# JADGardner/neusky

Hardware: AMD Instinct MI355X
Metric: train rays/sec on NeRF-OSR lk2 @1024 rays x 96 samples (higher is better)
Workload: dtype f32 in memory; forward products: fp16 hi + residual split, 3 x v_mfma_f32_32x32x16_f16 per product on power-of-two pre-scaled operands, one fp32 accumulator (~2^-22): FiLM-SIREN chains and the SDF / albedo field alike; backward products: the same fp16 split on per-row / per-matrix pre-scaled gradien; 1 GPU; full NeuSky train step (BASELINE configs[2]): 1024 rays/GPU x 96 samples, proposal 256+96, 512 illumination directions (256 upper-hemisphere DDF queries/ray), illumination decoder = this project's FiLM-SIREN H = 128 (RENI-shaped: latent 100x3; the reference's configured Attention decoder is absent from its tree), hash L16 F2 T2^19 x2, 256-wide MLPs; fwd + losses + bwd + all-reduce + 5 Adam groups; rays_per_gpu=1024, samples_per_ray=96, illumination_directions=512, parallelism=ray-sharded dp1, launcher=self-spawned, launch=HIP graph replay (1 graph/step + all-reduce + 5 Adam launches)

## Files before the change

### include/neusky_hip.h

```cpp
#ifndef NEUSKY_HIP_H
#define NEUSKY_HIP_H

#include <stdint.h>

#ifdef __cplusplus
extern "C" {
#endif

typedef void* nsky_stream_t;

const char* nsky_last_error(void);
int nsky_abi_version(void);

enum {
  NSKY_EPI_NONE = 0,
  NSKY_EPI_RELU = 1,
  NSKY_EPI_LEAKY = 2,
  NSKY_EPI_SIGMOID = 3,
  NSKY_EPI_SOFTPLUS = 4,
  NSKY_EPI_FILM = 5,
  NSKY_EPI_MUL_AUX = 6,
  NSKY_EPI_BWD_RELU = 7,
  NSKY_EPI_BWD_LEAKY = 8,
  NSKY_EPI_BWD_FILM = 9,
  NSKY_EPI_EXP = 10
};

enum { NSKY_PREC_F32 = 0, NSKY_PREC_BF16X2 = 2, NSKY_PREC_BF16X3 = 3, NSKY_PREC_F16X2 = 4 };

typedef struct nsky_gemm_desc {
  const float* A; const float* B; float* C;
  int32_t M, N, K;
  int32_t lda, ldb, ldc;
  int32_t a_kcontig, b_kcontig;
  const float* bias;
  int32_t epi;
  float p0, p1;
  const float* aux0; int32_t ldaux0;
  const float* aux1; int32_t ldaux1;
  const float* aux2; int32_t ldaux2;
  float* out1; int32_t ldout1;
  float* out2; int32_t ldout2;
  int32_t row_mod;
  int32_t k_splits;
  float beta;
  float* a_rowsum;
  int32_t precision;
  int32_t rowsum_k_limit;
  int32_t a_native_nt, b_native_nt;
  const float* a_scale_max;
} nsky_gemm_desc;

int nsky_gemm_f32(const nsky_gemm_desc* d, nsky_stream_t stream);

int nsky_split_planes(const float* W, int32_t n_rows, int32_t n_k, int32_t ldw, int32_t transpose, int32_t precision,
                      uint16_t* hi, uint16_t* lo, int32_t rows_pad, int32_t ldp, nsky_stream_t stream);
int nsky_gemm_f32_planes(const nsky_gemm_desc* d, const uint16_t* B_hi, const uint16_t* B_lo, int32_t ldp, nsky_stream_t stream);

int nsky_colsum_f32(const float* X, int32_t M, int32_t N, int32_t ldx, float* out, nsky_stream_t stream);
int nsky_weighted_colsum_f32(const float* X, int32_t M, int32_t N, int32_t ldx, const float* w, int32_t w_stride, float* out,
                             nsky_stream_t stream);

#define NSKY_FILM_MAX_LAYERS 12
#define NSKY_FILM_TABLE_FLOATS 6656
typedef struct nsky_film_net {
  int32_t hidden, n_map, n_film;
  int32_t cond_dim, x_dim, out_dim;
  const float* map_w[NSKY_FILM_MAX_LAYERS]; const float* map_b[NSKY_FILM_MAX_LAYERS]; int32_t map_ld[NSKY_FILM_MAX_LAYERS];
  const float* mo_w; const float* mo_b; int32_t mo_ld;
  const float* film_w[NSKY_FILM_MAX_LAYERS]; const float* film_b[NSKY_FILM_MAX_LAYERS]; int32_t film_ld[NSKY_FILM_MAX_LAYERS];
  const float* out_w; const float* out_b; int32_t out_ld;
} nsky_film_net;
int nsky_film_stream_layout(const nsky_film_net* net, int32_t direction, int64_t* stream_bytes, int32_t* n_tiles);
int nsky_film_pack(const nsky_film_net* net, int32_t direction, void* stream_buf, float* table, nsky_stream_t stream);
int nsky_film_chain_fwd(const nsky_film_net* net, const void* stream_buf, const float* table, const float* cond,
                        int32_t ldcond, const float* x, int32_t ldx, int32_t M, float* const* h_save, float* const* z_save,
                        float* const* y_save, float* res, int32_t ldres, nsky_stream_t stream);
int nsky_film_chain_bwd_film(const nsky_film_net* net, const void* stream_buf, const float* table, int32_t M, const float* d_res,
                             int32_t ldres, const float* h_last, const float* const* z_save, float* const* dz_save, float* dfp,
                             float* dfp_rowmax, float* gmax, float* d_x, int32_t ldx, nsky_stream_t stream);
int nsky_film_chain_bwd_map(const nsky_film_net* net, const void* stream_buf, const float* table, int32_t M, const float* dfp,
                            const float* dfp_rowmax, const float* const* h_save, float* const* dpre_save, float* d_cond,
                            int32_t ldcond, float* gmax, nsky_stream_t stream);
typedef struct {
  int32_t in_dim, hidden;
  const float* w0; int32_t ld0; const float* b0;
  const float* w1; int32_t ld1; const float* b1;
  const float* w2; const float* b2;
  float beta;
} nsky_sdf_net;
int nsky_sdf_stream_layout(const nsky_sdf_net* net, int32_t direction, int64_t* stream_bytes, int32_t* n_tiles);
int nsky_sdf_pack(const nsky_sdf_net* net, int32_t direction, void* stream_buf, float* table, nsky_stream_t stream);
int nsky_sdf_chain_fwd(const nsky_sdf_net* net, const void* stream_buf, const float* table, const float* E, int32_t ldE, int32_t M,
                       float* a0_save, float* a1_save, float* sdf, nsky_stream_t stream);
int nsky_sdf_chain_bwd(const nsky_sdf_net* net, const void* stream_buf, const float* table, int32_t M, const float* g_sdf,
                       const float* a0_save, const float* a1_save, float* dz1, float* dz0, float* dE, int32_t ldE, float* dw2,
                       float* db2, float* gmax, nsky_stream_t stream);

int nsky_wgrad_native(const float* dZ, int32_t nnt_a, const float* X, int32_t nnt_b, int32_t rows, float* dW, int32_t ldw,
                      float* db, const float* a_scale_max, float b_scale, nsky_stream_t stream);
#define NSKY_WGRAD_MAX_PROBLEMS 16
typedef struct {
  const float* dZ; int32_t nnt_a;
  const float* X;  int32_t nnt_b;
  float* dW;       int32_t ldw;
  float* db;
  const float* a_scale_max;
  float b_scale;
  int32_t lda, ldb, width_a, width_b, bias_rows;
  int32_t bias_row_mod;
  const float* b_scale_max;
} nsky_wgrad_problem;
int nsky_wgrad_native_batch(const nsky_wgrad_problem* problems, int32_t n_problems, int32_t rows, nsky_stream_t stream);

#define NSKY_CHAIN_MAX_LAYERS 8
typedef struct { const float* W; int32_t ld, rows, K, transposed; } nsky_chain_layer;
int nsky_chain_stream_layout(const nsky_chain_layer* layers, int32_t n_layers, int64_t* stream_bytes, int32_t* n_tiles, int32_t* n_groups);
int nsky_chain_pack(const nsky_chain_layer* layers, int32_t n_layers, void* stream_buf, float* scales, nsky_stream_t stream);
typedef struct nsky_field_net {
  int32_t in_dim;
  int32_t npe;
  float beta;
  const float* b0; const float* b1;
  const float* w_sdf; const float* b_sdf;
  const float* b2f;
  const float* bc0; const float* bc1;
  const float* wc2; int32_t ldc2; const float* bc2;
} nsky_field_net;
int nsky_field_geo_fwd(const nsky_field_net* net, const void* stream_buf, const float* scales, int32_t total_groups, const float* ET,
                       int32_t ldE, int32_t N, float* a0q, float* a1q, float* Eq, float* a1max, float* sdf, float* grad, float* qmax,
                       nsky_stream_t stream);
int nsky_field_colour_fwd(const nsky_field_net* net, const void* stream_buf, const float* scales, int32_t total_groups, const float* ET,
                          int32_t ldE, int32_t N, const float* a1q, const float* a1max, float* a1v, float* feat, float* xpe, float* c0, float* c1,
                          float* alb, nsky_stream_t stream);
int nsky_field_colour_bwd(const nsky_field_net* net, const void* stream_buf, const float* scales, int32_t total_groups, int32_t N,
                          const float* g_alb, const float* alb, const float* c0, const float* c1, float* dpc2, float* dpc1, float* dpc0,
                          float* dfeat, float* dxpe, float* da1v, float* gmax, nsky_stream_t stream);
int nsky_field_geo_bwd(const nsky_field_net* net, const void* stream_buf, const float* scales, int32_t total_groups, int32_t N,
                       const float* g_sdf, const float* g_grad, const float* da1v, const float* dxpe, const float* a0q, const float* a1q,
                       float* d1q, float* d0q, float* dET, int32_t ldE, float* gmax, nsky_stream_t stream);
int nsky_native_weighted_colsum(const float* X, int32_t nt, int32_t rows, const float* w4, int32_t n_out, const float* g_sdf,
                                const float* g_grad, float* out, int32_t ldo, float* bias, nsky_stream_t stream);
int nsky_field_geo_fwd_dir(const nsky_field_net* net, const void* stream_buf, const float* scales, int32_t total_groups, const float* ET,
                           int32_t ldE, int32_t N, float* a0q, float* a1q, float* Eq, float* sdf, float* cosv, float* qmax,
                           nsky_stream_t stream);
int nsky_field_geo_bwd_dir(const nsky_field_net* net, const void* stream_buf, const float* scales, int32_t total_groups, int32_t N,
                           const float* g_sdf, const float* g_cos, const float* a0q, const float* a1q, float* d1q, float* d0q, float* dET,
                           int32_t ldE, float* gmax, nsky_stream_t stream);
int nsky_native_weighted_colsum_pair(const float* X, int32_t nt, int32_t rows, const float* g_sdf, const float* g_cos, float* out,
                                     int32_t ldo, float* bias, nsky_stream_t stream);

int nsky_ray_reduce_fwd(const float* weights, const float* starts, const float* ends, const float* normals, const float* albedo,
                        int32_t R, int32_t S, float max_clamp, float* sums, float* bounds, float* p2p, float* accumulation,
                        float* normal, float* albedo_acc, nsky_stream_t stream);
int nsky_ray_reduce_bwd(const float* weights, const float* starts, const float* ends, const float* normals, const float* albedo,
                        const float* sums, const float* bounds, int32_t R, int32_t S, float max_clamp, const float* d_p2p,
                        const float* d_accumulation, const float* d_normal, const float* d_albedo_acc, float* d_weights,
                        float* d_normals, float* d_albedo, nsky_stream_t stream);


int nsky_point_alphas_fwd(const float* sdf, const float* grad, const float* dirs, const float* gap3_host, const float* variance, float anneal,
                          int32_t P, float* alphas, nsky_stream_t stream);
int nsky_point_alphas_bwd(const float* sdf, const float* grad, const float* dirs, const float* gap3_host, const float* variance, float anneal,
                          int32_t P, const float* d_alphas, float* d_sdf, float* d_grad, float* d_variance, nsky_stream_t stream);

int nsky_sigmoid_column_fwd(const float* raw, int32_t ld, int64_t n, float scale, float* t, nsky_stream_t stream);
int nsky_sigmoid_column_bwd(const float* raw, int32_t ld, int64_t n, float scale, const float* d_t, float* d_raw, nsky_stream_t stream);

int nsky_proposal_mlp_fwd(const float* feat, int32_t ldf, int64_t P, int32_t in_dim, int32_t hidden, const float* w0, int32_t ldw0,
                          const float* b0, const float* w1, const float* b1, float* raw, nsky_stream_t stream);
int nsky_proposal_mlp_bwd(const float* feat, int32_t ldf, int64_t P, int32_t in_dim, int32_t hidden, const float* w0, int32_t ldw0,
                          const float* b0, const float* w1, const float* b1, const float* d_raw, float* d_feat, float* dw0, float* db0,
                          float* dw1, float* db1, nsky_stream_t stream);
int nsky_ray_points_fwd(const float* origins, const float* dirs, int32_t n_dirs, float sign, const float* t, int64_t n, float* out,
                        nsky_stream_t stream);
int nsky_ray_points_bwd(const float* dirs, int32_t n_dirs, float sign, const float* d_out, int64_t n, float* d_t, nsky_stream_t stream);
int nsky_normalize3_fwd(const float* g, int64_t P, float* n, nsky_stream_t stream);
int nsky_normalize3_bwd(const float* g, const float* d_n, int64_t P, float* d_g, nsky_stream_t stream);

int nsky_ddf_vmf_samples(int32_t n_positions, int32_t n_directions, float kappa, float radius, int32_t upper_hemisphere,
                         uint64_t seed, uint64_t* counter, float* origins, float* directions, nsky_stream_t stream);

int nsky_ddf_fit_rows_fwd(const float* positions, const float* directions, const float* term_dist, int32_t N,
                          const float* mv_points_in, uint64_t seed, uint64_t* counter, const float* sky_o, const float* sky_d,
                          int32_t Ns, float radius, int32_t want_mv, float weight_exp, int32_t weight_include_z, float* q_pos,
                          float* xrow, int32_t ldx, float* mv_points_out, float* sky_gt, float* distance_weight, nsky_stream_t stream);
int nsky_ddf_fit_rows_bwd(const float* positions, const float* directions, const float* term_dist, const float* mv_points,
                          int32_t N, const float* d_xrow_mv, int32_t ldx, float* d_term_dist, nsky_stream_t stream);


int nsky_grid_probe_points(const float* lattice, const float* gap3_host, int32_t P, uint64_t seed, uint64_t* counter, float* positions,
                           float* directions, nsky_stream_t stream);

int nsky_reni_output_fwd(const float* raw, int32_t ldr, const float* scale, const int64_t* ray_latent, int32_t U, int32_t D, int32_t R,
                         float* grid, float* rays, nsky_stream_t stream);
int nsky_reni_output_bwd(const float* raw, int32_t ldr, const float* scale, const int64_t* ray_latent, int32_t U, int32_t D, int32_t R,
                         const float* d_grid, const float* d_rays, float* d_raw, float* d_scale, nsky_stream_t stream);

int nsky_illumination_directions(const float* base, int32_t D, const float* rotation_in, uint64_t seed, uint64_t* counter, float* dirs,
                                 int32_t* sel, float* rot_out, nsky_stream_t stream);
int nsky_reni_grid_inputs_fwd(const float* latents, const float* directions, int32_t U, int32_t L, int32_t D, const float* ray_dirs,
                              const int64_t* ray_latent, int32_t R, float* cond, int32_t ldcond, float* xrow, int32_t ldx,
                              nsky_stream_t stream);
int nsky_reni_grid_inputs_bwd(const float* latents, const float* directions, int32_t U, int32_t L, int32_t D, const float* ray_dirs,
                              const int64_t* ray_latent, int32_t R, const float* d_cond, int32_t ldcond, float* d_latents,
                              nsky_stream_t stream);

typedef struct nsky_hashgrid_desc {
  const float* table;
  int32_t n_levels;
  int32_t smoothstep;
  float scale[16];
  int32_t resolution[16];
  uint32_t offset[17];
} nsky_hashgrid_desc;

int nsky_encode_fwd(const nsky_hashgrid_desc* g, const float* x, int32_t P, int32_t mode, int32_t include_x,
                    int32_t pe_freqs, float pe_max_exp, float* Y, int32_t ldy, float* T, nsky_stream_t stream);

#define NSKY_ENCODE_BWD_OWNER_MIN_POINTS 32768
int64_t nsky_encode_bwd_workspace_bytes(const nsky_hashgrid_desc* g, int32_t P, int32_t tangents);
int nsky_encode_bwd(const nsky_hashgrid_desc* g, const float* x, int32_t P, int32_t mode, int32_t include_x,
                    int32_t pe_freqs, float pe_max_exp, const float* dY, int32_t lddy, const float* dT, float* dtable,
                    float* dx, void* workspace, nsky_stream_t stream);
int nsky_encode_fwd_dir(const nsky_hashgrid_desc* g, const float* x, int32_t P, int32_t mode, int32_t include_x, int32_t pe_freqs,
                        float pe_max_exp, const float* dirs, int32_t spr, float* Y, int32_t ldy, float* Td, nsky_stream_t stream);
int nsky_encode_bwd_dir(const nsky_hashgrid_desc* g, const float* x, int32_t P, int32_t mode, int32_t include_x, int32_t pe_freqs,
                        float pe_max_exp, const float* dirs, int32_t spr, const float* dY, int32_t lddy, const float* dTd,
                        float* dtable, void* workspace, nsky_stream_t stream);

int nsky_hash_indices(const nsky_hashgrid_desc* g, const float* x, int32_t P, int32_t mode, uint32_t* idx,
                      nsky_stream_t stream);

int nsky_hemi_composite_fwd(const float* albedo, const float* normals, const float* weights, const float* dirs,
                            const float* cam_colours, const int32_t* cam_of_ray, const float* vis, const float* bg,
                            int32_t R, int32_t S, int32_t D, float* rgb, float* lin, nsky_stream_t stream);
// ... 284 lines not shown
```

### neusky_amd/csrc/film_chain.hip

```cpp
#include "chain.h"

namespace {

constexpr int FWD_FRAG_BUFFERS = 3;


struct Layout {
  int NT, Gc, Gx, Gh;
  long base_map, base_film0, base_film, base_head, total_groups;
  int n_tiles;
};

__host__ __device__ inline Layout fwd_layout(const nsky_film_net& n) {
  Layout L;
  L.NT = n.hidden / 32;
  L.Gc = groups_of(n.cond_dim);
  L.Gx = groups_of(n.x_dim);
  L.Gh = groups_of(n.hidden);
  L.base_map = (long)L.NT * L.Gc;
  L.base_film0 = L.base_map + (long)(n.n_map - 1) * L.NT * L.Gh;
  L.base_film = L.base_film0 + (long)L.NT * (2 * L.Gh + L.Gx);
  L.base_head = L.base_film + (long)(n.n_film - 1) * L.NT * 3 * L.Gh;
  L.total_groups = L.base_head + L.Gh;
  L.n_tiles = n.n_map * L.NT + n.n_film * L.NT * 3 + 1;
  return L;
}


__device__ inline TileDesc fwd_tile(const nsky_film_net& n, const Layout& L, int idx) {
  TileDesc d;
  d.transposed = 0;
  d.k0 = 0;
  const int NT = L.NT, H = n.hidden;
  if (idx < NT) {
    d.W = n.map_w[0]; d.ld = n.map_ld[0]; d.row0 = 32 * idx; d.nrows = 32; d.K = n.cond_dim; d.group = (long)idx * L.Gc;
    return d;
  }
  idx -= NT;
  if (idx < (n.n_map - 1) * NT) {
    const int l = 1 + idx / NT, t = idx % NT;
    d.W = n.map_w[l]; d.ld = n.map_ld[l]; d.row0 = 32 * t; d.nrows = 32; d.K = H; d.group = L.base_map + (long)idx * L.Gh;
    return d;
  }
  idx -= (n.n_map - 1) * NT;
  if (idx < n.n_film * NT * 3) {
    const int i = idx / (3 * NT), t = (idx / 3) % NT, which = idx % 3;
    const long tb = i == 0 ? L.base_film0 + (long)t * (2 * L.Gh + L.Gx) : L.base_film + ((long)(i - 1) * NT + t) * 3 * L.Gh;
    d.nrows = 32;
    if (which < 2) {
      d.W = n.mo_w; d.ld = n.mo_ld; d.row0 = (which == 0 ? i : n.n_film + i) * H + 32 * t; d.K = H; d.group = tb + which * L.Gh;
    } else {
      d.W = n.film_w[i]; d.ld = n.film_ld[i]; d.row0 = 32 * t; d.K = i == 0 ? n.x_dim : H; d.group = tb + 2 * L.Gh;
    }
    return d;
  }
  d.W = n.out_w; d.ld = n.out_ld; d.row0 = 0; d.nrows = n.out_dim; d.K = H; d.group = L.base_head;
  return d;
}

__host__ __device__ inline void bwd_film_layout(const nsky_film_net& n, long& total_groups, int& n_tiles) {
  const int NT = n.hidden / 32, Gh = groups_of(n.hidden);
  n_tiles = n.n_film * NT * 2 + (n.n_film - 1) * NT + 1;
  total_groups = (long)n_tiles * Gh;
}
__host__ __device__ inline void bwd_map_layout(const nsky_film_net& n, long& total_groups, int& n_tiles) {
  const int NT = n.hidden / 32, Gh = groups_of(n.hidden);
  const int nkb = 2 * n.n_film * n.hidden / 64, ct = (n.cond_dim + 31) / 32;
  n_tiles = nkb * NT + (n.n_map - 1) * NT + ct;
  total_groups = (long)nkb * (NT / 2) + (long)((n.n_map - 1) * NT + ct) * Gh;
}

__device__ inline TileDesc bwd_film_tile(const nsky_film_net& n, int idx) {
  TileDesc d;
  const int NT = n.hidden / 32, H = n.hidden, Gh = groups_of(H);
  d.group = (long)idx * Gh;
  d.nrows = 32; d.K = H; d.k0 = 0; d.transposed = 0;
  if (idx == n.n_film * NT * 2 + (n.n_film - 1) * NT) {
    d.W = n.film_w[0]; d.ld = n.film_ld[0]; d.row0 = 0; d.nrows = n.x_dim; d.transposed = 1;
    return d;
  }
  int i = n.n_film - 1, rem = idx;
  while (i > 0 && rem >= 3 * NT) { rem -= 3 * NT; --i; }
  if (rem < 2 * NT) {
    const int t = rem / 2, which = rem % 2;
    d.W = n.mo_w; d.ld = n.mo_ld; d.row0 = (which == 0 ? i : n.n_film + i) * H + 32 * t;
  } else {
    const int u = rem - 2 * NT;
    d.W = n.film_w[i]; d.ld = n.film_ld[i]; d.row0 = 32 * u; d.transposed = 1;
  }
  return d;
}

__device__ inline TileDesc bwd_map_tile(const nsky_film_net& n, int idx) {
  TileDesc d;
  const int NT = n.hidden / 32, H = n.hidden, Gh = groups_of(H);
  const int nkb = 2 * n.n_film * H / 64;
  d.nrows = 32; d.transposed = 1; d.k0 = 0;
  if (idx < nkb * NT) {
    const int kb = idx / NT, u = idx % NT;
    d.W = n.mo_w; d.ld = n.mo_ld; d.row0 = 32 * u; d.K = 64; d.k0 = 64 * kb; d.group = idx / 2; d.slab0 = 4 * (u & 1);
    return d;
  }
  idx -= nkb * NT;
  d.group = (long)nkb * (NT / 2) + (long)idx * Gh;
  d.K = H;
  if (idx < (n.n_map - 1) * NT) {
    const int l = n.n_map - 1 - idx / NT, u = idx % NT;
    d.W = n.map_w[l]; d.ld = n.map_ld[l]; d.row0 = 32 * u;
    return d;
  }
  idx -= (n.n_map - 1) * NT;
  d.W = n.map_w[0]; d.ld = n.map_ld[0]; d.row0 = 32 * idx; d.nrows = min(32, n.cond_dim - 32 * idx);
  return d;
}

__host__ __device__ inline void dir_layout(const nsky_film_net& n, int direction, long& total_groups, int& n_tiles) {
  if (direction == 0) { const Layout L = fwd_layout(n); total_groups = L.total_groups; n_tiles = L.n_tiles; }
  else if (direction == 1) bwd_film_layout(n, total_groups, n_tiles);
  else bwd_map_layout(n, total_groups, n_tiles);
}

__device__ inline void write_bias_table(const nsky_film_net& n, float* bl, int tid) {
  const int H = n.hidden;
  int off = 0;
  for (int l = 0; l < n.n_map; ++l, off += H)
    for (int i = tid; i < H; i += 256) bl[off + i] = n.map_b[l] ? n.map_b[l][i] : 0.0f;
  for (int i = tid; i < 2 * n.n_film * H; i += 256) bl[off + i] = n.mo_b ? n.mo_b[i] : 0.0f;
  off += 2 * n.n_film * H;
  for (int l = 0; l < n.n_film; ++l, off += H)
    for (int i = tid; i < H; i += 256) bl[off + i] = n.film_b[l] ? n.film_b[l][i] : 0.0f;
  for (int i = tid; i < 32; i += 256) bl[off + i] = (n.out_b && i < n.out_dim) ? n.out_b[i] : 0.0f;
}


__global__ __launch_bounds__(256) void film_pack_kernel(nsky_film_net net, int direction, unsigned char* __restrict__ stream,
                                                        float* __restrict__ table) {
  __shared__ float w[32][PACK_KMAX + 1];
  __shared__ float red[256];
  const int tid = threadIdx.x;
  long total_groups;
  int n_tiles;
  dir_layout(net, direction, total_groups, n_tiles);
  if ((int)blockIdx.x == n_tiles) {
    write_bias_table(net, table, tid);
    return;
  }
  const TileDesc d = direction == 0 ? fwd_tile(net, fwd_layout(net), blockIdx.x)
                                    : (direction == 1 ? bwd_film_tile(net, blockIdx.x) : bwd_map_tile(net, blockIdx.x));
  pack_tile(d, stream, table + BIAS_FLOATS, w, red);
}



struct FwdArgs {
  nsky_film_net net;
  const unsigned char* stream;
  const float* table;
  const float* cond; int ldcond;
  const float* x; int ldx;
  int M;
  float* h_save[MAXL];
  float* z_save[MAXL];
  float* y_save[MAXL];
  float* res; int ldres;
};


template <int H, int KSC, bool KEEP_Y = true>
__global__ __launch_bounds__(256, 1) void film_fwd_kernel(const FwdArgs a) {
  constexpr int NT = H / 32, KS = H / 16;
  __shared__ __attribute__((aligned(16))) unsigned char smem[RING_BYTES + (BIAS_FLOATS + SCALE_FLOATS) * 4];
  float* bl = reinterpret_cast<float*>(smem + RING_BYTES);
  const nsky_film_net& net = a.net;
  const int tid = threadIdx.x, lane = tid & 63;
  const int wave = __builtin_amdgcn_readfirstlane(tid >> 6);
  const int c = lane & 31, h = lane >> 5;
  float* sl = bl + BIAS_FLOATS;
  NSKY_STAGE_TABLE((BIAS_FLOATS + SCALE_FLOATS) / 4, 256, a.table, bl, tid);
  __syncthreads();
  WStream ws;
  ws_open<4, false, RING_GROUPS, true>(ws, a.stream, smem, wave, lane);

  const long rt = (long)blockIdx.x * 4 + wave;
  const long row = rt * 32 + c;
  const bool live = row < a.M;
  const long rowc = live ? row : a.M - 1;
  const bool wave_live = rt * 32 < a.M;
  const int n_map = net.n_map, n_film = net.n_film;
  int tile = 0;

  f16x8 hh[KS], hl[KS];
  float h_inv;
  {
    f16x8 ch[KSC], cl[KSC];
    const int ksc = ksteps_of(net.cond_dim);
    const float c_inv = load_planes<KSC>(a.cond + rowc * a.ldcond, (net.cond_dim + 3) & ~3, ksc, h, ch, cl);
    float hn[NT][16];
    float m = 0.0f;
#pragma unroll
    for (int t = 0; t < NT; ++t) {
      f32x16 acc;
#pragma unroll
      for (int r = 0; r < 16; ++r) acc[r] = 0.0f;
      product_dyn<KSC>(ws, ksc, ch, cl, acc);
      const float inv = c_inv * sl[tile++];
#pragma unroll
      for (int g = 0; g < 4; ++g) {
        const float4 b = *reinterpret_cast<const float4*>(bl + 32 * t + 8 * g + 4 * h);
        const float bb[4] = {b.x, b.y, b.z, b.w};
#pragma unroll
        for (int q = 0; q < 4; ++q) {
          const float v = fmaf(acc[4 * g + q], inv, bb[q]);
          const float o = v > 0.0f ? v : 0.2f * v;
          hn[t][4 * g + q] = o;
          m = fmaxf(m, fabsf(o));
        }
      }
      if (a.h_save[0] && wave_live) store_tile_nt(a.h_save[0] + (rt * NT + t) * 1024, lane, hn[t]);
    }
    const float s = row_scale(m, h_inv);
#pragma unroll
    for (int t = 0; t < NT; ++t)
#pragma unroll
      for (int u = 0; u < 2; ++u) {
        float x8[8];
#pragma unroll
        for (int j = 0; j < 8; ++j) x8[j] = hn[t][8 * u + j] * s;
        split8(x8, hh[2 * t + u], hl[2 * t + u]);
      }
  }
  for (int l = 1; l < n_map; ++l) {
    float hn[NT][16];
    float m = 0.0f;
    const float* bias = bl + l * H;
#pragma unroll
    for (int t = 0; t < NT; ++t) {
      f32x16 acc;
#pragma unroll
      for (int r = 0; r < 16; ++r) acc[r] = 0.0f;
      product<KS, 4, false, RING_GROUPS, FWD_FRAG_BUFFERS>(ws, hh, hl, acc);
      const float inv = h_inv * sl[tile++];
#pragma unroll
      for (int g = 0; g < 4; ++g) {
        const float4 b = *reinterpret_cast<const float4*>(bias + 32 * t + 8 * g + 4 * h);
        const float bb[4] = {b.x, b.y, b.z, b.w};
#pragma unroll
        for (int q = 0; q < 4; ++q) {
          const float v = fmaf(acc[4 * g + q], inv, bb[q]);
          const float o = v > 0.0f ? v : 0.2f * v;
          hn[t][4 * g + q] = o;
          m = fmaxf(m, fabsf(o));
        }
      }
      if (a.h_save[l] && wave_live) store_tile_nt(a.h_save[l] + (rt * NT + t) * 1024, lane, hn[t]);
    }
    const float s = row_scale(m, h_inv);
#pragma unroll
    for (int t = 0; t < NT; ++t)
#pragma unroll
      for (int u = 0; u < 2; ++u) {
        float x8[8];
#pragma unroll
        for (int j = 0; j < 8; ++j) x8[j] = hn[t][8 * u + j] * s;
        split8(x8, hh[2 * t + u], hl[2 * t + u]);
      }
  }
  f16x8 xh[1], xl[1];
  const float x_inv = load_planes<1>(a.x + rowc * a.ldx, (net.x_dim + 3) & ~3, 1, h, xh, xl);
  f16x8 yh[KS], yl[KS];
#pragma unroll
  for (int ks = 0; ks < KS; ++ks)
#pragma unroll
    for (int j = 0; j < 8; ++j) { yh[ks][j] = (_Float16)0.0f; yl[ks][j] = (_Float16)0.0f; }
  const float* bias_mo = bl + n_map * H;
  const float* bias_film = bias_mo + 2 * n_film * H;
  for (int i = 0; i < n_film; ++i) {
    const float* bF = bias_mo + i * H;
    const float* bP = bias_mo + (n_film + i) * H;
    const float* bZ = bias_film + i * H;
    float* zblk = a.z_save[i] ? a.z_save[i] + (wave_live ? rt : 0) * NT * 1024 : nullptr;
    float* yblk = KEEP_Y ? a.y_save[i] + (wave_live ? rt : 0) * NT * 1024 : nullptr;
    f16x8 nh[KEEP_Y ? 1 : KS], nl[KEEP_Y ? 1 : KS];
    for (int t = 0; t < NT; ++t) {
      f32x16 aF, aP, aZ;
#pragma unroll
      for (int r = 0; r < 16; ++r) { aF[r] = 0.0f; aP[r] = 0.0f; aZ[r] = 0.0f; }
      product<KS, 4, false, RING_GROUPS, FWD_FRAG_BUFFERS>(ws, hh, hl, aF);
      product<KS, 4, false, RING_GROUPS, FWD_FRAG_BUFFERS>(ws, hh, hl, aP);
      float z_unscale;
      if (i == 0) {
        product<1>(ws, xh, xl, aZ);
        z_unscale = x_inv;
      } else {
        product<KS, 4, false, RING_GROUPS, FWD_FRAG_BUFFERS>(ws, yh, yl, aZ);
        z_unscale = 1.0f / Y_SCALE;
      }
      const float iF = h_inv * sl[tile], iP = h_inv * sl[tile + 1], iZ = z_unscale * sl[tile + 2];
      tile += 3;
      float zz[16], yy[16];
#pragma unroll
      for (int g = 0; g < 4; ++g) {
        const int fo = 32 * t + 8 * g + 4 * h;
        const float4 b4F = *reinterpret_cast<const float4*>(bF + fo);
        const float4 b4P = *reinterpret_cast<const float4*>(bP + fo);
        const float4 b4Z = *reinterpret_cast<const float4*>(bZ + fo);
        const float bf[4] = {b4F.x, b4F.y, b4F.z, b4F.w}, bp[4] = {b4P.x, b4P.y, b4P.z, b4P.w}, bz[4] = {b4Z.x, b4Z.y, b4Z.z, b4Z.w};
#pragma unroll
        for (int q = 0; q < 4; ++q) {
          const int r = 4 * g + q;
          const float F = fmaf(aF[r], iF, bf[q]), P = fmaf(aP[r], iP, bp[q]), z = fmaf(aZ[r], iZ, bz[q]);
          zz[r] = z;
          yy[r] = sin_cw(fmaf(fmaf(15.0f, F, 30.0f), z, P));
        }
      }
      if (wave_live) {
        if (zblk) store_tile_nt(zblk + t * 1024, lane, zz);
        if constexpr (KEEP_Y) store_tile(yblk + t * 1024, lane, yy);
      }
      if constexpr (!KEEP_Y) {
#pragma unroll
        for (int tt = 0; tt < NT; ++tt)
          if (t == tt) {
#pragma unroll
            for (int u = 0; u < 2; ++u) {
              float x8[8];
#pragma unroll
              for (int j = 0; j < 8; ++j) x8[j] = yy[8 * u + j] * Y_SCALE;
              split8(x8, nh[2 * tt + u], nl[2 * tt + u]);
            }
          }
      }
    }
    if constexpr (!KEEP_Y) {
#pragma unroll
      for (int ks = 0; ks < KS; ++ks) { yh[ks] = nh[ks]; yl[ks] = nl[ks]; }
      continue;
    }
#pragma unroll
    for (int ks = 0; ks < KS; ++ks) {
      float x8[8];
#pragma unroll
      for (int u = 0; u < 2; ++u) {
        const float4 q = ldg4_nt(yblk + (ks >> 1) * 1024 + (2 * (ks & 1) + u) * 256 + lane * 4);
        x8[4 * u] = q.x * Y_SCALE; x8[4 * u + 1] = q.y * Y_SCALE; x8[4 * u + 2] = q.z * Y_SCALE; x8[4 * u + 3] = q.w * Y_SCALE;
      }
      split8(x8, yh[ks], yl[ks]);
    }
  }

  {
    f32x16 acc;
#pragma unroll
    for (int r = 0; r < 16; ++r) acc[r] = 0.0f;
    product<KS, 4, false, RING_GROUPS, FWD_FRAG_BUFFERS>(ws, yh, yl, acc);
    const float inv = sl[tile] / Y_SCALE;
    const float* bO = bias_film + n_film * H;
    if (live && h == 0)
      stg4(a.res + row * a.ldres, make_float4(fmaf(acc[0], inv, bO[0]), fmaf(acc[1], inv, bO[1]), fmaf(acc[2], inv, bO[2]),
                                              fmaf(acc[3], inv, bO[3])));
  }
  ws_close();
}


struct BwdFilmArgs {
  nsky_film_net net;
  const unsigned char* stream;
  const float* table;
  int M;
  const float* d_res; int ldres;
  const float* h_last;
  const float* z_save[MAXL];
  float* dz_save[MAXL];
  float* dfp;
  float* dfp_rowmax;
  float* gmax;
  float* d_x; int ldx;
  int full_wgs, tail_wgs, tail_k;
};


template <int OFF>
__device__ __forceinline__ void hidden_load4_s(f32x4& q, const float* sbase, int voff) {
  asm volatile("global_load_dwordx4 %0, %1, %2 offset:%3" : "+v"(q) : "v"(voff), "s"(sbase), "n"(OFF) : "memory");
}

template <int H, bool ACTIVE, bool KEEP>
__device__ __forceinline__ void film_bwd4_tile(const BwdFilmArgs& a, WStream& ws, const float* bl, const float* sl, const float* wo, long rt, int lane) {
  constexpr int NT = H / 32, KS = H / 16, GH = (KS + GSLABS - 1) / GSLABS, PW = 4;
  const nsky_film_net& net = a.net;
  const int c = lane & 31, h = lane >> 5;
  const long row = rt * 32 + c;
  const bool live = ACTIVE && row < a.M;
  const long rowc = row < a.M ? row : a.M - 1;
  const int n_film = net.n_film;
  f32x16 dY[NT];
  float h_inv = 1.0f, h_scale = 1.0f;
  if (ACTIVE) {
    float m = 0.0f;
    for (int t = 0; t < NT; ++t) {
      float hv[16];
      load_tile(a.h_last + (rt * NT + t) * 1024, lane, hv);
#pragma unroll
      for (int r = 0; r < 16; ++r) m = fmaxf(m, fabsf(hv[r]));
    }
    h_scale = row_scale(m, h_inv);
    const float4 dr = ldg4(a.d_res + rowc * a.ldres);
#pragma unroll
    for (int t = 0; t < NT; ++t)
#pragma unroll
      for (int g = 0; g < 4; ++g) {
        const int fo = 32 * t + 8 * g + 4 * h;
        const float4 w0 = *reinterpret_cast<const float4*>(wo + fo), w1 = *reinterpret_cast<const float4*>(wo + H + fo);
        const float4 w2 = *reinterpret_cast<const float4*>(wo + 2 * H + fo), w3 = *reinterpret_cast<const float4*>(wo + 3 * H + fo);
        dY[t][4 * g] = dr.x * w0.x + dr.y * w1.x + dr.z * w2.x + dr.w * w3.x;
        dY[t][4 * g + 1] = dr.x * w0.y + dr.y * w1.y + dr.z * w2.y + dr.w * w3.y;
        dY[t][4 * g + 2] = dr.x * w0.z + dr.y * w1.z + dr.z * w2.z + dr.w * w3.z;
        dY[t][4 * g + 3] = dr.x * w0.w + dr.y * w1.w + dr.z * w2.w + dr.w * w3.w;
      }
  } else {
#pragma unroll
    for (int t = 0; t < NT; ++t)
#pragma unroll
      for (int r = 0; r < 16; ++r) dY[t][r] = 0.0f;
  }
  const float* bias_mo = bl + net.n_map * H;
  float fp_max = 0.0f;
  int tile = 0;
  constexpr bool H_RESIDENT = H <= 128;
  f16x8 hh[KS], hl[KS];
  auto load_h = [&]() {
    int hoff = 0;
    asm volatile("" : "+s"(hoff));
#pragma unroll
    for (int t = 0; t < NT; ++t) {
      float hv[16];
      load_tile(a.h_last + ((rt * NT + t) * 1024 + hoff), lane, hv);
#pragma unroll
      for (int u = 0; u < 2; ++u) {
        float x8[8];
#pragma unroll
        for (int j = 0; j < 8; ++j) x8[j] = hv[8 * u + j] * h_scale;
        split8(x8, hh[2 * t + u], hl[2 * t + u]);
      }
    }
    asm volatile("s_waitcnt vmcnt(0)" ::: "memory");
  };
  if (ACTIVE && H_RESIDENT) load_h();
  for (int i = n_film - 1; i >= 0; --i) {
    const float* bF = bias_mo + i * H;
    const float* bP = bias_mo + (n_film + i) * H;
    const float* zp = a.z_save[i] + rt * NT * 1024;
    float* dzp = KEEP ? a.dz_save[i] + rt * NT * 1024 : nullptr;
    float* dFp = a.dfp + (rt * (2 * n_film * NT) + (long)i * NT) * 1024;
    float* dPp = a.dfp + (rt * (2 * n_film * NT) + (long)(n_film + i) * NT) * 1024;
    float dz_max = 0.0f;
    {
      if (ACTIVE && !H_RESIDENT) load_h();
#pragma unroll
      for (int t = 0; t < NT; ++t) {
        f32x4 zq[4];
        int toff = t * 1024;
        asm volatile("" : "+s"(toff));
        const float* zpt = zp + toff;
        float *dzt = dzp + toff, *dFt = dFp + toff, *dPt = dPp + toff;
        if (ACTIVE) {
#pragma unroll
          for (int g = 0; g < 4; ++g) zq[g] = f32x4{0.f, 0.f, 0.f, 0.f};
          hidden_load4_s<0>(zq[0], zpt, lane * 16);
          hidden_load4_s<1024>(zq[1], zpt, lane * 16);
          hidden_load4_s<2048>(zq[2], zpt, lane * 16);
          hidden_load4_s<3072>(zq[3], zpt, lane * 16);
        }
        f32x16 aF, aP;
        prod<KS, PW>(ws, ACTIVE, hh, hl, aF);
        prod<KS, PW>(ws, ACTIVE, hh, hl, aP);
        if (ACTIVE) {
          hidden_wait<2 * GH * PW>(zq);
          const float iF = h_inv * sl[tile], iP = h_inv * sl[tile + 1];
#pragma unroll
          for (int g = 0; g < 4; ++g) {
            const int fo = 32 * t + 8 * g + 4 * h;
            const float4 b4F = *reinterpret_cast<const float4*>(bF + fo);
            const float4 b4P = *reinterpret_cast<const float4*>(bP + fo);
            const float bf[4] = {b4F.x, b4F.y, b4F.z, b4F.w}, bp[4] = {b4P.x, b4P.y, b4P.z, b4P.w};
            float dzv[4], dFv[4], dPv[4];
#pragma unroll
            for (int q = 0; q < 4; ++q) {
              const int r = 4 * g + q;
              const float F = fmaf(aF[r], iF, bf[q]), P = fmaf(aP[r], iP, bp[q]), z = zq[g][q];
              const float f = fmaf(15.0f, F, 30.0f);
              const float gc = dY[t][r] * cos_cw(fmaf(f, z, P));
              dzv[q] = gc * f;
              dFv[q] = 15.0f * gc * z;
              dPv[q] = gc;
              dY[t][r] = dzv[q];
              dz_max = fmaxf(dz_max, fabsf(dzv[q]));
              fp_max = fmaxf(fp_max, fmaxf(fabsf(dFv[q]), fabsf(gc)));
            }
            if constexpr (KEEP) {
              stg4(dzt + (g * 256 + lane * 4), make_float4(dzv[0], dzv[1], dzv[2], dzv[3]));
              stg4(dFt + (g * 256 + lane * 4), make_float4(dFv[0], dFv[1], dFv[2], dFv[3]));
              stg4(dPt + (g * 256 + lane * 4), make_float4(dPv[0], dPv[1], dPv[2], dPv[3]));
            } else {
              *reinterpret_cast<f32x4*>(dFt + (g * 256 + lane * 4)) = f32x4{dFv[0], dFv[1], dFv[2], dFv[3]};
              *reinterpret_cast<f32x4*>(dPt + (g * 256 + lane * 4)) = f32x4{dPv[0], dPv[1], dPv[2], dPv[3]};
            }
            asm volatile("" : "+v"(dz_max), "+v"(fp_max));
          }
        }
        tile += 2;
      }
    }
    {
      float dz_inv = 1.0f;
      f16x8 dh_[KS], dl_[KS];
      if (ACTIVE) {
        if constexpr (KEEP) publish_max(a.gmax + i, dz_max, live, true, lane);
        const float s = row_scale(dz_max, dz_inv);
#pragma unroll
        for (int ks = 0; ks < KS; ++ks) {
          float x8[8];
#pragma unroll
          for (int j = 0; j < 8; ++j) x8[j] = dY[ks >> 1][8 * (ks & 1) + j] * s;
          split8(x8, dh_[ks], dl_[ks]);
        }
      }
      if (i > 0) {
#pragma unroll
        for (int u = 0; u < NT; ++u) {
          f32x16 acc;
          prod<KS, PW>(ws, ACTIVE, dh_, dl_, acc);
          if (ACTIVE) {
            const float inv = dz_inv * sl[tile];
#pragma unroll
            for (int r = 0; r < 16; ++r) dY[u][r] = acc[r] * inv;
          }
          ++tile;
        }
      } else {
        f32x16 acc;
        prod<KS, PW>(ws, ACTIVE, dh_, dl_, acc);
        if (ACTIVE && a.d_x && live) {
          const float inv = dz_inv * sl[tile];
#pragma unroll
          for (int g = 0; g < 2; ++g)
            if (8 * g + 4 * h < ((net.x_dim + 3) & ~3))
              stg4(a.d_x + row * a.ldx + 8 * g + 4 * h, make_float4(acc[4 * g] * inv, acc[4 * g + 1] * inv, acc[4 * g + 2] * inv, acc[4 * g + 3] * inv));
        }
        ++tile;
      }
    }
  }
  if (ACTIVE) {
    fp_max = fmaxf(fp_max, __shfl_xor(fp_max, 32, 64));
    if (h == 0) a.dfp_rowmax[row] = fp_max;
    publish_max(a.gmax + n_film, fp_max, live, true, lane);
  }
}

template <int H, bool KEEP = true>
__global__ __launch_bounds__(256, 1) void film_bwd4_kernel(const BwdFilmArgs a) {
  __shared__ __attribute__((aligned(16))) unsigned char smem[RING_BYTES + (BIAS_FLOATS + SCALE_FLOATS) * 4 + 4 * H * 4];
  float* bl = reinterpret_cast<float*>(smem + RING_BYTES);
  float* sl = bl + BIAS_FLOATS;
  float* wo = sl + SCALE_FLOATS;
  const nsky_film_net& net = a.net;
  const int tid = threadIdx.x, lane = tid & 63;
  const int wave = __builtin_amdgcn_readfirstlane(tid >> 6);
  NSKY_STAGE_TABLE((BIAS_FLOATS + SCALE_FLOATS) / 4, 256, a.table, bl, tid);
  for (int i = tid; i < 4 * H; i += 256) wo[i] = (i / H) < net.out_dim ? net.out_w[(long)(i / H) * net.out_ld + (i % H)] : 0.0f;
  __syncthreads();
  WStream ws;
  ws_open(ws, a.stream, smem, wave, lane);
  const long n_tiles = (a.M + 31) / 32;
  const long rt = (long)blockIdx.x * 4 + wave;
  if (rt < n_tiles) film_bwd4_tile<H, true, KEEP>(a, ws, bl, sl, wo, rt, lane);
  else film_bwd4_tile<H, false, KEEP>(a, ws, bl, sl, wo, 0, lane);
  ws_close();
}

struct BwdMapArgs {
  nsky_film_net net;
  const unsigned char* stream;
  const float* table;
  int M;
  const float* dfp;
  const float* dfp_rowmax;
  const float* h_save[MAXL];
  float* dpre_save[MAXL];
  float* d_cond; int ldcond;
  float* gmax;
  int full_wgs, tail_wgs, tail_k;
};

template <int H, bool ACTIVE, bool KEEP>
__device__ __forceinline__ void film_bwd_map_tile(const BwdMapArgs& a, WStream& ws, const float* sl, long rt, int lane) {
  constexpr int NT = H / 32, KS = H / 16, PW = 2;
  constexpr bool REGS = !KEEP && H <= 128;
  float dreg[REGS ? NT : 1][16];
  const nsky_film_net& net = a.net;
  const int c = lane & 31, h = lane >> 5;
  const long row = rt * 32 + c;
  const bool live = ACTIVE && row < a.M;
  const int nkb = 2 * net.n_film * H / 64, ntot = 2 * net.n_film * NT;
  float f_inv = 1.0f, f_scale = 1.0f;
  if (ACTIVE) f_scale = row_scale(a.dfp_rowmax[rt * 32 + c], f_inv);
  int tile = 0;
  const float* fblk = a.dfp + rt * ntot * 1024;
  const int top = net.n_map - 1;
  float m = 0.0f;
  f32x4 fq[8];
#define NSKY_FQ_WAIT(N)                                                                                                         \
  asm volatile("s_waitcnt vmcnt(%8)"                                                                                            \
               : "+v"(fq[0]), "+v"(fq[1]), "+v"(fq[2]), "+v"(fq[3]), "+v"(fq[4]), "+v"(fq[5]), "+v"(fq[6]), "+v"(fq[7])           \
               : "n"(N)                                                                                                         \
               : "memory")
  f32x16 dh[NT];
#pragma unroll
  for (int u = 0; u < NT; ++u)
#pragma unroll
    for (int r = 0; r < 16; ++r) dh[u][r] = 0.0f;
  if (ACTIVE) {
#pragma unroll
    for (int j = 0; j < 8; ++j) fq[j] = f32x4{0.f, 0.f, 0.f, 0.f};
#pragma unroll
    for (int j = 0; j < 8; ++j) hidden_load4(fq[j], fblk + (j >> 2) * 1024 + (j & 3) * 256 + lane * 4);
    NSKY_FQ_WAIT(0);
  }
  for (int kb = 0; kb < nkb; ++kb) {
    f16x8 ph[4], pl[4];
    if (ACTIVE) {
#pragma unroll
      for (int ks = 0; ks < 4; ++ks) {
        float x8[8];
#pragma unroll
        for (int u = 0; u < 2; ++u) {
          const f32x4 q = fq[(ks >> 1) * 4 + 2 * (ks & 1) + u];
          x8[4 * u] = q[0] * f_scale; x8[4 * u + 1] = q[1] * f_scale; x8[4 * u + 2] = q[2] * f_scale; x8[4 * u + 3] = q[3] * f_scale;
        }
        split8(x8, ph[ks], pl[ks]);
      }
      const int kn = kb + 1 < nkb ? kb + 1 : kb;
#pragma unroll
      for (int j = 0; j < 8; ++j) hidden_load4(fq[j], fblk + (long)(2 * kn + (j >> 2)) * 1024 + (j & 3) * 256 + lane * 4);
    }
#pragma unroll
    for (int v = 0; v < NT / 2; ++v) {
      if (ACTIVE) {
        if (kb > 0) {
#pragma unroll
          for (int e = 0; e < 2; ++e) {
            const float ratio = __int_as_float(__float_as_int(sl[tile + e - NT]) - __float_as_int(sl[tile + e]) + 0x3f800000);
            if (ratio != 1.0f)
#pragma unroll
              for (int r = 0; r < 16; ++r) dh[2 * v + e][r] *= ratio;
          }
        }
        product_pair<PW>(ws, ph, pl, dh[2 * v], dh[2 * v + 1]);
      } else {
        product_skip<8, PW, false>(ws);
      }
      tile += 2;
    }
    if (ACTIVE) NSKY_FQ_WAIT(PW * (NT / 2));
  }
  if (ACTIVE) {
#pragma unroll
    for (int u = 0; u < NT; ++u) {
      const float inv = f_inv * sl[tile - NT + u];
      float hv[16], dv[16];
      load_tile(a.h_save[top] + (rt * NT + u) * 1024, lane, hv);
#pragma unroll
      for (int r = 0; r < 16; ++r) {
        const float g = dh[u][r] * inv;
        dv[r] = hv[r] > 0.0f ? g : 0.2f * g;
        m = fmaxf(m, fabsf(dv[r]));
      }
      if constexpr (REGS) {
#pragma unroll
        for (int r = 0; r < 16; ++r) dreg[u][r] = dv[r];
      } else {
        store_tile(a.dpre_save[top] + (rt * NT + u) * 1024, lane, dv);
      }
    }
    asm volatile("s_waitcnt vmcnt(0)" ::: "memory");
  }
#undef NSKY_FQ_WAIT

  for (int l = top; l >= 0; --l) {
    float d_inv = 1.0f;
    f16x8 ph[KS], pl[KS];
    if (ACTIVE) {
      if constexpr (KEEP) publish_max(a.gmax + l, m, live, true, lane);
      const float s = row_scale(m, d_inv);
#pragma unroll
      for (int u = 0; u < NT; ++u) {
        float dv[16];
        if constexpr (REGS) {
#pragma unroll
          for (int r = 0; r < 16; ++r) dv[r] = dreg[u][r];
        } else {
          load_tile(a.dpre_save[l] + (rt * NT + u) * 1024, lane, dv);
        }
#pragma unroll
        for (int v = 0; v < 2; ++v) {
          float x8[8];
#pragma unroll
          for (int j = 0; j < 8; ++j) x8[j] = dv[8 * v + j] * s;
          split8(x8, ph[2 * u + v], pl[2 * u + v]);
        }
      }
      asm volatile("s_waitcnt vmcnt(0)" ::: "memory");
    }
    m = 0.0f;
    if (l > 0) {
      for (int u = 0; u < NT; ++u) {
        f32x16 acc;
        prod<KS, PW>(ws, ACTIVE, ph, pl, acc);
        if (ACTIVE) {
          const float inv = d_inv * sl[tile];
          float hv[16], dv[16];
          load_tile(a.h_save[l - 1] + (rt * NT + u) * 1024, lane, hv);
#pragma unroll
          for (int r = 0; r < 16; ++r) {
            const float g = acc[r] * inv;
            dv[r] = hv[r] > 0.0f ? g : 0.2f * g;
            m = fmaxf(m, fabsf(dv[r]));
          }
          if constexpr (REGS) {
#pragma unroll
            for (int uu = 0; uu < NT; ++uu)
              if (u == uu) {
#pragma unroll
                for (int r = 0; r < 16; ++r) dreg[uu][r] = dv[r];
              }
          } else {
            store_tile(a.dpre_save[l - 1] + (rt * NT + u) * 1024, lane, dv);
          }
          asm volatile("s_waitcnt vmcnt(0)" ::: "memory");
        }
        ++tile;
      }
    } else {
      const int ct = (net.cond_dim + 31) / 32;
      for (int u = 0; u < ct; ++u) {
        f32x16 acc;
        prod<KS, PW>(ws, ACTIVE, ph, pl, acc);
        if (ACTIVE && a.d_cond && live) {
          const float inv = d_inv * sl[tile];
#pragma unroll
          for (int g = 0; g < 4; ++g) {
            const int fo = 32 * u + 8 * g + 4 * h;
            if (fo < ((net.cond_dim + 3) & ~3))
              stg4(a.d_cond + row * a.ldcond + fo, make_float4(acc[4 * g] * inv, acc[4 * g + 1] * inv, acc[4 * g + 2] * inv, acc[4 * g + 3] * inv));
          }
        }
        ++tile;
      }
    }
  }
}

template <int H, bool KEEP = true>
__global__ __launch_bounds__(512, 2) void film_bwd_map_kernel(const BwdMapArgs a) {
  constexpr int PW = 2;
  __shared__ __attribute__((aligned(16))) unsigned char smem[RING_BYTES + SCALE_FLOATS * 4];
  float* sl = reinterpret_cast<float*>(smem + RING_BYTES);
  const int tid = threadIdx.x, lane = tid & 63;
  const int wave = __builtin_amdgcn_readfirstlane(tid >> 6);
  for (int i = tid; i < SCALE_FLOATS; i += 512) sl[i] = a.table[BIAS_FLOATS + i];
  __syncthreads();
  WStream ws;
  ws_open<PW>(ws, a.stream, smem, wave, lane);
  const long n_tiles = (a.M + 31) / 32;
  const long rt = tail_tile(a.full_wgs, a.tail_wgs, a.tail_k, n_tiles, wave);
  if (rt >= 0 && rt < n_tiles) film_bwd_map_tile<H, true, KEEP>(a, ws, sl, rt, lane);
  else film_bwd_map_tile<H, false, KEEP>(a, ws, sl, 0, lane);
  ws_close();
}

int check_net(const nsky_film_net* n, const char* who) {
  NSKY_CHECK_ARG(n, "%s: null network", who);
  NSKY_CHECK_ARG(n->hidden == 128 || n->hidden == 256, "%s: hidden width %d (128 or 256)", who, n->hidden);
  NSKY_CHECK_ARG(n->n_map >= 1 && n->n_map <= MAXL && n->n_film >= 1 && n->n_film <= MAXL, "%s: layer counts %d / %d", who, n->n_map, n->n_film);
  NSKY_CHECK_ARG(n->cond_dim >= 1 && n->cond_dim <= PACK_KMAX && n->x_dim >= 1 && n->x_dim <= 16 && n->out_dim >= 1 && n->out_dim <= 4,
                 "%s: cond_dim %d (<= %d), x_dim %d (<= 16), out_dim %d (<= 4)", who, n->cond_dim, PACK_KMAX, n->x_dim, n->out_dim);
  const int nb = n->n_map * n->hidden + 3 * n->n_film * n->hidden + 32;
  NSKY_CHECK_ARG(nb <= BIAS_FLOATS, "%s: %d bias values exceed the LDS table (%d)", who, nb, BIAS_FLOATS);
  NSKY_CHECK_ARG(fwd_layout(*n).n_tiles <= SCALE_FLOATS, "%s: %d weight tiles exceed the LDS scale table (%d)", who, fwd_layout(*n).n_tiles, SCALE_FLOATS);
  for (int l = 0; l < n->n_map; ++l) NSKY_CHECK_ARG(n->map_w[l] && n->map_ld[l] >= (l == 0 ? n->cond_dim : n->hidden), "%s: mapping layer %d", who, l);
  for (int l = 0; l < n->n_film; ++l) NSKY_CHECK_ARG(n->film_w[l] && n->film_ld[l] >= (l == 0 ? n->x_dim : n->hidden), "%s: FiLM layer %d", who, l);
  NSKY_CHECK_ARG(n->mo_w && n->mo_ld >= n->hidden && n->out_w && n->out_ld >= n->hidden, "%s: head weights", who);
  return NSKY_OK;
}

}

extern "C" int nsky_film_stream_layout(const nsky_film_net* net, int32_t direction, int64_t* stream_bytes, int32_t* n_tiles) {
  if (int rc = check_net(net, "nsky_film_stream_layout")) return rc;
  NSKY_CHECK_ARG(direction >= 0 && direction <= 2, "nsky_film_stream_layout: direction %d", direction);
  long groups;
  int tiles;
  dir_layout(*net, direction, groups, tiles);
  NSKY_CHECK_ARG(tiles <= SCALE_FLOATS, "nsky_film_stream_layout: %d weight tiles exceed the scale table (%d)", tiles, SCALE_FLOATS);
  if (stream_bytes) *stream_bytes = (groups + RING_GROUPS + 2) * (int64_t)GROUP;
  if (n_tiles) *n_tiles = tiles;
  return NSKY_OK;
}

extern "C" int nsky_film_pack(const nsky_film_net* net, int32_t direction, void* stream_buf, float* table, nsky_stream_t stream) {
  if (int rc = check_net(net, "nsky_film_pack")) return rc;
  NSKY_CHECK_ARG(direction >= 0 && direction <= 2 && stream_buf && table && ((uintptr_t)stream_buf % 16) == 0 && ((uintptr_t)table % 16) == 0, "nsky_film_pack: bad arguments");
  long groups;
  int tiles;
  dir_layout(*net, direction, groups, tiles);
  NSKY_CHECK_ARG(tiles <= SCALE_FLOATS, "nsky_film_pack: %d weight tiles exceed the scale table (%d)", tiles, SCALE_FLOATS);
  if (direction != 0) NSKY_CHECK_ARG(net->hidden % 128 == 0, "nsky_film_pack: backward streams need hidden %% 128 == 0");
  hipLaunchKernelGGL(film_pack_kernel, dim3(tiles + 1), dim3(256), 0, (hipStream_t)stream, *net, direction, (unsigned char*)stream_buf, table);
  NSKY_CHECK_LAUNCH("nsky_film_pack");
  return NSKY_OK;
}

extern "C" int nsky_film_chain_fwd(const nsky_film_net* net, const void* stream_buf, const float* table, const float* cond,
                                   int32_t ldcond, const float* x, int32_t ldx, int32_t M, float* const* h_save, float* const* z_save,
                                   float* const* y_save, float* res, int32_t ldres, nsky_stream_t stream) {
  if (int rc = check_net(net, "nsky_film_chain_fwd")) return rc;
  NSKY_CHECK_ARG(stream_buf && table && cond && x && res && M > 0, "nsky_film_chain_fwd: null operand / empty batch");
  NSKY_CHECK_ARG(ldcond % 4 == 0 && ldcond >= ((net->cond_dim + 3) & ~3) && ldx % 4 == 0 && ldx >= ((net->x_dim + 3) & ~3) && ldres >= 4 && ldres % 4 == 0,
                 "nsky_film_chain_fwd: leading dimensions (cond %d, x %d, res %d) must be multiples of 4 covering the padded widths", ldcond, ldx, ldres);
  NSKY_CHECK_ARG(((uintptr_t)cond % 16) == 0 && ((uintptr_t)x % 16) == 0 && ((uintptr_t)res % 16) == 0 && ((uintptr_t)stream_buf % 16) == 0 && ((uintptr_t)table % 16) == 0,
                 "nsky_film_chain_fwd: operands must be 16-byte aligned");
  FwdArgs a;
  a.net = *net;
  a.stream = (const unsigned char*)stream_buf; a.table = table;
  a.cond = cond; a.ldcond = ldcond; a.x = x; a.ldx = ldx; a.M = M; a.res = res; a.ldres = ldres;
  for (int l = 0; l < MAXL; ++l) {
    a.h_save[l] = (h_save && l < net->n_map) ? h_save[l] : nullptr;
    a.z_save[l] = (z_save && l < net->n_film) ? z_save[l] : nullptr;
    a.y_save[l] = (y_save && l < net->n_film) ? y_save[l] : nullptr;
  }
  const bool keep_y = a.y_save[0] != nullptr;
  NSKY_CHECK_ARG(keep_y || net->hidden == 128, "nsky_film_chain_fwd: NULL y_save needs hidden 128 (hidden %d: pass two ping-pong buffers)", net->hidden);
  for (int l = 0; l < net->n_film; ++l)
    NSKY_CHECK_ARG((a.y_save[l] != nullptr) == keep_y && ((uintptr_t)a.y_save[l] % 16) == 0, "nsky_film_chain_fwd: y_save[%d] missing / unaligned", l);
  const dim3 grid(ceil_div(M, 128));
  const int ksc = ksteps_of(net->cond_dim);
#define NSKY_FILM_FWD(HH, KK, KEEP) hipLaunchKernelGGL((film_fwd_kernel<HH, KK, KEEP>), grid, dim3(256), 0, (hipStream_t)stream, a)
  if (net->hidden == 256) { if (ksc <= 4) NSKY_FILM_FWD(256, 4, true); else NSKY_FILM_FWD(256, 20, true); }
  else if (keep_y) { if (ksc <= 4) NSKY_FILM_FWD(128, 4, true); else NSKY_FILM_FWD(128, 20, true); }
  else { if (ksc <= 4) NSKY_FILM_FWD(128, 4, false); else NSKY_FILM_FWD(128, 20, false); }
#undef NSKY_FILM_FWD
  NSKY_CHECK_LAUNCH("nsky_film_chain_fwd");
  return NSKY_OK;
}


extern "C" int nsky_film_chain_bwd_film(const nsky_film_net* net, const void* stream_buf, const float* table, int32_t M, const float* d_res,
                                        int32_t ldres, const float* h_last, const float* const* z_save, float* const* dz_save, float* dfp,
                                        float* dfp_rowmax, float* gmax, float* d_x, int32_t ldx, nsky_stream_t stream) {
  if (int rc = check_net(net, "nsky_film_chain_bwd_film")) return rc;
  NSKY_CHECK_ARG(stream_buf && table && d_res && h_last && z_save && dfp && dfp_rowmax && gmax && M > 0, "nsky_film_chain_bwd_film: null operand / empty batch");
  NSKY_CHECK_ARG(ldres >= 4 && ldres % 4 == 0 && ((uintptr_t)d_res % 16) == 0 && ((uintptr_t)h_last % 16) == 0 && ((uintptr_t)dfp % 16) == 0 &&
                     ((uintptr_t)stream_buf % 16) == 0 && ((uintptr_t)table % 16) == 0, "nsky_film_chain_bwd_film: alignment / ldres");
  NSKY_CHECK_ARG(net->hidden % 128 == 0, "nsky_film_chain_bwd_film: hidden %% 128");
  BwdFilmArgs a;
  a.net = *net; a.stream = (const unsigned char*)stream_buf; a.table = table; a.M = M; a.d_res = d_res; a.ldres = ldres; a.h_last = h_last;
  a.dfp = dfp; a.dfp_rowmax = dfp_rowmax; a.gmax = gmax; a.d_x = d_x; a.ldx = ldx;
  if (d_x) NSKY_CHECK_ARG(ldx % 4 == 0 && ldx >= ((net->x_dim + 3) & ~3) && ldx <= 16 && ((uintptr_t)d_x % 16) == 0, "nsky_film_chain_bwd_film: d_x layout (ldx %d)", ldx);
  for (int l = 0; l < MAXL; ++l) {
    a.z_save[l] = l < net->n_film ? z_save[l] : nullptr;
    a.dz_save[l] = (dz_save && l < net->n_film) ? dz_save[l] : nullptr;
  }
  const bool keep = a.dz_save[0] != nullptr;
  for (int l = 0; l < net->n_film; ++l)
    NSKY_CHECK_ARG(a.z_save[l] && (a.dz_save[l] != nullptr) == keep && ((uintptr_t)a.z_save[l] % 16) == 0 && ((uintptr_t)a.dz_save[l] % 16) == 0, "nsky_film_chain_bwd_film: z_save / dz_save[%d]", l);
  a.full_wgs = a.tail_wgs = a.tail_k = 0;
  const dim3 grid(ceil_div(ceil_div(M, 32), 4));
#define NSKY_FILM_BWD4(HH, KEEP) hipLaunchKernelGGL((film_bwd4_kernel<HH, KEEP>), grid, dim3(256), 0, (hipStream_t)stream, a)
  if (net->hidden == 256) { if (keep) NSKY_FILM_BWD4(256, true); else NSKY_FILM_BWD4(256, false); }
  else { if (keep) NSKY_FILM_BWD4(128, true); else NSKY_FILM_BWD4(128, false); }
#undef NSKY_FILM_BWD4
  NSKY_CHECK_LAUNCH("nsky_film_chain_bwd_film");
  return NSKY_OK;
}

extern "C" int nsky_film_chain_bwd_map(const nsky_film_net* net, const void* stream_buf, const float* table, int32_t M, const float* dfp,
                                       const float* dfp_rowmax, const float* const* h_save, float* const* dpre_save, float* d_cond,
                                       int32_t ldcond, float* gmax, nsky_stream_t stream) {
  if (int rc = check_net(net, "nsky_film_chain_bwd_map")) return rc;
  NSKY_CHECK_ARG(stream_buf && table && dfp && dfp_rowmax && h_save && gmax && M > 0, "nsky_film_chain_bwd_map: null operand / empty batch");
  NSKY_CHECK_ARG(((uintptr_t)dfp % 16) == 0 && ((uintptr_t)stream_buf % 16) == 0 && ((uintptr_t)table % 16) == 0, "nsky_film_chain_bwd_map: alignment");
  if (d_cond) NSKY_CHECK_ARG(ldcond % 4 == 0 && ldcond >= ((net->cond_dim + 3) & ~3) && ((uintptr_t)d_cond % 16) == 0, "nsky_film_chain_bwd_map: d_cond layout");
  NSKY_CHECK_ARG(net->hidden % 128 == 0, "nsky_film_chain_bwd_map: hidden %% 128");
  BwdMapArgs a;
  a.net = *net; a.stream = (const unsigned char*)stream_buf; a.table = table; a.M = M; a.dfp = dfp; a.dfp_rowmax = dfp_rowmax;
  a.d_cond = d_cond; a.ldcond = ldcond; a.gmax = gmax;
  for (int l = 0; l < MAXL; ++l) {
    a.h_save[l] = l < net->n_map ? h_save[l] : nullptr;
    a.dpre_save[l] = (dpre_save && l < net->n_map) ? dpre_save[l] : nullptr;
  }
  const bool regs = a.dpre_save[0] == nullptr;
  const bool keep = !regs && !(net->n_map > 1 && a.dpre_save[1] == a.dpre_save[0]);
  NSKY_CHECK_ARG(!regs || net->hidden == 128, "nsky_film_chain_bwd_map: NULL dpre_save needs hidden 128 (hidden %d: pass one shared buffer)", net->hidden);
  for (int l = 0; l < net->n_map; ++l)
    NSKY_CHECK_ARG(a.h_save[l] && (a.dpre_save[l] == nullptr) == regs && (keep || a.dpre_save[l] == a.dpre_save[0]) && ((uintptr_t)a.h_save[l] % 16) == 0 &&
                       ((uintptr_t)a.dpre_save[l] % 16) == 0, "nsky_film_chain_bwd_map: h_save / dpre_save[%d]", l);
  const TailPlan tp = tail_plan(ceil_div(M, 32), device_cus());
  a.full_wgs = tp.full_wgs; a.tail_wgs = tp.tail_wgs; a.tail_k = tp.tail_k;
  const dim3 grid(tp.full_wgs + tp.tail_wgs);
#define NSKY_FILM_BWD_MAP(HH, KEEP) hipLaunchKernelGGL((film_bwd_map_kernel<HH, KEEP>), grid, dim3(512), 0, (hipStream_t)stream, a)
  if (net->hidden == 256) { if (keep) NSKY_FILM_BWD_MAP(256, true); else NSKY_FILM_BWD_MAP(256, false); }
  else { if (keep) NSKY_FILM_BWD_MAP(128, true); else NSKY_FILM_BWD_MAP(128, false); }
#undef NSKY_FILM_BWD_MAP
  NSKY_CHECK_LAUNCH("nsky_film_chain_bwd_map");
  return NSKY_OK;
}
```

### neusky_amd/hip.py

```python
from __future__ import annotations

import ctypes as C
import os

import torch

_HERE = os.path.dirname(os.path.abspath(__file__))
LIB_PATH = os.path.join(_HERE, "libneusky_hip.so")


class NeuSkyHipError(RuntimeError):
    pass


if not os.path.exists(LIB_PATH):
    raise ImportError(
        f"{LIB_PATH} not found: build the HIP extension first (python -c 'import __graft_entry__ as g; g.build()'). "
        "neusky_amd has no CPU/PyTorch fallback."
    )
_lib = C.CDLL(LIB_PATH)

EPI_NONE, EPI_RELU, EPI_LEAKY, EPI_SIGMOID, EPI_SOFTPLUS, EPI_FILM, EPI_MUL_AUX = 0, 1, 2, 3, 4, 5, 6
EPI_BWD_RELU, EPI_BWD_LEAKY, EPI_BWD_FILM, EPI_EXP = 7, 8, 9, 10
PREC_F32, PREC_BF16X2, PREC_BF16X3, PREC_F16X2 = 0, 2, 3, 4
# ... 506 lines not shown


def density_weights_bwd(raw, ebins, d_weights, d_raw):
    R, n = d_weights.shape
    check(_dw_bwd(ptr(raw), ld(raw), _c(ebins), _c(d_weights), R, n, _c(d_raw), stream_ptr()), "nsky_density_weights_bwd")
    return d_raw


def weight_norm_fwd(v, g, row_map, col_map, out, inv_norm):
    check(_wn_fwd(ptr(v), ptr(g), row_map.numel(), col_map.numel(), v.shape[1], ld(v), ptr(row_map), ptr(col_map), ptr(out),
                  ld(out), ptr(inv_norm), stream_ptr()), "nsky_weight_norm_fwd")
    return out


def weight_norm_bwd(d_out, v, g, inv_norm, row_map, inverse_col, dv, dg):
    check(_wn_bwd(ptr(d_out), ld(d_out), ptr(v), ptr(g), ptr(inv_norm), row_map.numel(), v.shape[1], ld(v), ptr(row_map),
                  ptr(inverse_col), ptr(dv), ptr(dg), stream_ptr()), "nsky_weight_norm_bwd")


def adam_step(p, g, m, v, lr, beta1, beta2, eps, step, grad_scale=1.0):
    n = p.numel()
    assert p.is_contiguous() and g.is_contiguous() and m.is_contiguous() and v.is_contiguous()
    check(_adam(ptr(p), ptr(g), ptr(m), ptr(v), n, lr, beta1, beta2, eps, step, grad_scale, stream_ptr()), "nsky_adam_step")


_attn_fwd = _sig("nsky_attn_core_fwd", C.c_void_p, C.c_void_p, C.c_void_p, C.c_void_p, C.c_int32, C.c_int32, C.c_int32, C.c_int32, C.c_float,
                 C.c_void_p, C.c_void_p, C.c_void_p, C.c_void_p)
_attn_bwd = _sig("nsky_attn_core_bwd", C.c_void_p, C.c_void_p, C.c_void_p, C.c_void_p, C.c_void_p, C.c_void_p, C.c_void_p, C.c_void_p,
                 C.c_int32, C.c_int32, C.c_int32, C.c_int32, C.c_float, C.c_void_p, C.c_void_p, C.c_void_p, C.c_void_p, C.c_void_p)
_add_ln_fwd = _sig("nsky_add_layer_norm_fwd", C.c_void_p, C.c_void_p, C.c_void_p, C.c_void_p, C.c_int64, C.c_int32, C.c_float, C.c_void_p, C.c_void_p,
                   C.c_void_p, C.c_void_p)
_add_ln_bwd = _sig("nsky_add_layer_norm_bwd", C.c_void_p, C.c_void_p, C.c_void_p, C.c_void_p, C.c_void_p, C.c_int64, C.c_int32, C.c_void_p, C.c_void_p)


def add_layer_norm_fwd(x, r, gamma, beta, eps, s, y, stats):
    M, W = x.shape
    assert all(t is None or t.is_contiguous() for t in (x, r, gamma, beta, s, y, stats))
    check(_add_ln_fwd(ptr(x), ptr(r), ptr(gamma), ptr(beta), M, W, float(eps), ptr(s), ptr(y), ptr(stats), stream_ptr()), "nsky_add_layer_norm_fwd")


def add_layer_norm_bwd(s, stats, gamma, dy, ds_in, ds):
    M, W = s.shape
    assert all(t is None or t.is_contiguous() for t in (s, stats, gamma, dy, ds_in, ds))
    check(_add_ln_bwd(ptr(s), ptr(stats), ptr(gamma), ptr(dy), ptr(ds_in), M, W, ptr(ds), stream_ptr()), "nsky_add_layer_norm_bwd")


_attn_rays_fwd = _sig("nsky_attn_core_rays_fwd", C.c_void_p, C.c_void_p, C.c_void_p, C.c_void_p, C.c_void_p, C.c_void_p, C.c_int32, C.c_int32, C.c_int32,
                      C.c_int32, C.c_float, C.c_void_p, C.c_void_p, C.c_void_p, C.c_void_p)
_attn_rays_bwd = _sig("nsky_attn_core_rays_bwd", C.c_void_p, C.c_void_p, C.c_void_p, C.c_void_p, C.c_void_p, C.c_void_p, C.c_void_p, C.c_void_p,
                      C.c_void_p, C.c_void_p, C.c_int32, C.c_int32, C.c_int32, C.c_int32, C.c_float, C.c_void_p, C.c_void_p, C.c_void_p, C.c_void_p)


def attn_core_rays_fwd(Q, dirs, perm, seg, Kt, Vt, scale, O, row_max, row_sum):
    R, H = Q.shape
    U, nh, L = Kt.shape[0], Kt.shape[1], Kt.shape[2]
    assert H == 16 * nh and perm.dtype == torch.int32 and seg.dtype == torch.int32 and seg.numel() == U + 1
    assert all(t.is_contiguous() for t in (Q, dirs, perm, seg, Kt, Vt, O, row_max, row_sum))
    check(_attn_rays_fwd(ptr(Q), ptr(dirs), ptr(perm), ptr(seg), ptr(Kt), ptr(Vt), U, R, L, nh, float(scale), ptr(O), ptr(row_max), ptr(row_sum),
                         stream_ptr()), "nsky_attn_core_rays_fwd")
    return O


def attn_core_rays_bwd(Q, dirs, perm, seg, Kt, Vt, O, row_max, row_sum, dO, scale, dQ, dKt, dVt):
    R, H = Q.shape
    U, nh, L = Kt.shape[0], Kt.shape[1], Kt.shape[2]
    assert all(t.is_contiguous() for t in (Q, dirs, perm, seg, Kt, Vt, O, row_max, row_sum, dO, dQ, dKt, dVt))
    check(_attn_rays_bwd(ptr(Q), ptr(dirs), ptr(perm), ptr(seg), ptr(Kt), ptr(Vt), ptr(O), ptr(row_max), ptr(row_sum), ptr(dO), U, R, L, nh,
                         float(scale), ptr(dQ), ptr(dKt), ptr(dVt), stream_ptr()), "nsky_attn_core_rays_bwd")


def attn_core_fwd(Q, dirs, Kt, Vt, scale, O, row_max, row_sum):
    U, D, H = Q.shape
    nh, L = Kt.shape[1], Kt.shape[2]
    assert H == 16 * nh and Kt.shape[3] == 48 and all(t.is_contiguous() for t in (Q, dirs, Kt, Vt, O, row_max, row_sum))
    check(_attn_fwd(ptr(Q), ptr(dirs), ptr(Kt), ptr(Vt), U, D, L, nh, float(scale), ptr(O), ptr(row_max), ptr(row_sum), stream_ptr()),
          "nsky_attn_core_fwd")
    return O


def attn_core_bwd(Q, dirs, Kt, Vt, O, row_max, row_sum, dO, scale, dQ, dKt, dVt):
    U, D, H = Q.shape
    nh, L = Kt.shape[1], Kt.shape[2]
    assert all(t.is_contiguous() for t in (Q, dirs, Kt, Vt, O, row_max, row_sum, dO, dQ, dKt, dVt))
    drow = torch.empty(U * nh * (D + 4), device=Q.device)
    check(_attn_bwd(ptr(Q), ptr(dirs), ptr(Kt), ptr(Vt), ptr(O), ptr(row_max), ptr(row_sum), ptr(dO), U, D, L, nh, float(scale),
                    ptr(dQ), ptr(dKt), ptr(dVt), ptr(drow), stream_ptr()), "nsky_attn_core_bwd")


TOTAL_MAX_SEGMENTS = 8


class TotalSegment(C.Structure):
    _fields_ = [("x", C.c_void_p), ("coef", C.c_void_p), ("grad", C.c_void_p), ("n", C.c_int32), ("scale", C.c_float)]


_total_fwd = _sig("nsky_weighted_total_fwd", C.POINTER(TotalSegment), C.c_int32, C.c_void_p, C.c_void_p)
_total_bwd = _sig("nsky_weighted_total_bwd", C.POINTER(TotalSegment), C.c_int32, C.c_void_p, C.c_void_p)


def weighted_total_fwd(parts, total):
    assert 0 < len(parts) <= TOTAL_MAX_SEGMENTS
    arr = (TotalSegment * len(parts))(*[TotalSegment(ptr(x), ptr(c), None, x.numel(), float(sc)) for x, c, sc in parts])
    check(_total_fwd(arr, len(parts), ptr(total), stream_ptr()), "nsky_weighted_total_fwd")
    return total


def weighted_total_bwd(parts, g, grads):
    arr = (TotalSegment * len(parts))(*[TotalSegment(ptr(x), ptr(c), ptr(d), x.numel(), float(sc)) for (x, c, sc), d in zip(parts, grads)])
    check(_total_bwd(arr, len(parts), ptr(g), stream_ptr()), "nsky_weighted_total_bwd")


class MainLossesDesc(C.Structure):
    _fields_ = [("R", C.c_int32), ("S", C.c_int32), ("P", C.c_int32), ("M", C.c_int32),
                ("rgb", C.c_void_p), ("image", C.c_void_p), ("mask", C.c_void_p), ("eik", C.c_void_p), ("weights", C.c_void_p),
                ("normal", C.c_void_p), ("hdr_bg", C.c_void_p), ("grid", C.c_void_p), ("sdf_term", C.c_void_p), ("vis_thr", C.c_void_p),
                ("sky_alpha", C.c_float), ("vis_target", C.c_float)]


class DDFLossesDesc(C.Structure):
    _fields_ = [("Mr", C.c_int32), ("Mm", C.c_int32), ("Ms", C.c_int32),
                ("expected", C.c_void_p), ("term", C.c_void_p), ("mask", C.c_void_p), ("dist_weight", C.c_void_p), ("sdf", C.c_void_p),
                ("mv_expected", C.c_void_p), ("mv_term", C.c_void_p), ("sky_expected", C.c_void_p), ("sky_term", C.c_void_p),
                ("want_depth", C.c_int32), ("want_sdf_l2", C.c_int32), ("want_sdf_l1", C.c_int32), ("mask_to_circumference", C.c_int32),
                ("inverse_depth_weight", C.c_int32), ("radius", C.c_float)]


_main_losses_fwd = _sig("nsky_main_losses_fwd", C.POINTER(MainLossesDesc), C.c_void_p, C.c_void_p, C.c_void_p)
_main_losses_bwd = _sig("nsky_main_losses_bwd", C.POINTER(MainLossesDesc), *([C.c_void_p] * 11))
_ddf_losses_fwd = _sig("nsky_ddf_losses_fwd", C.POINTER(DDFLossesDesc), C.c_void_p, C.c_void_p)
_ddf_losses_bwd = _sig("nsky_ddf_losses_bwd", C.POINTER(DDFLossesDesc), *([C.c_void_p] * 8))
N_MAIN_TERMS, N_DDF_TERMS = 8, 5


def main_losses_fwd(desc: MainLossesDesc, terms, wsum):
    check(_main_losses_fwd(C.byref(desc), ptr(terms), ptr(wsum), stream_ptr()), "nsky_main_losses_fwd")


def main_losses_bwd(desc: MainLossesDesc, wsum, d_terms, d_rgb, d_eik, d_weights, d_normal, d_hdr_bg, d_grid, d_sdf_term, d_vis_thr):
    check(_main_losses_bwd(C.byref(desc), ptr(wsum), ptr(d_terms), ptr(d_rgb), ptr(d_eik), ptr(d_weights), ptr(d_normal), ptr(d_hdr_bg),
                           ptr(d_grid), ptr(d_sdf_term), ptr(d_vis_thr), stream_ptr()), "nsky_main_losses_bwd")


def ddf_losses_fwd(desc: DDFLossesDesc, terms):
    check(_ddf_losses_fwd(C.byref(desc), ptr(terms), stream_ptr()), "nsky_ddf_losses_fwd")


def ddf_losses_bwd(desc: DDFLossesDesc, d_terms, d_expected, d_sdf, d_mv_expected, d_sky_expected, d_term, d_mv_term):
    check(_ddf_losses_bwd(C.byref(desc), ptr(d_terms), ptr(d_expected), ptr(d_sdf), ptr(d_mv_expected), ptr(d_sky_expected), ptr(d_term),
                          ptr(d_mv_term), stream_ptr()), "nsky_ddf_losses_bwd")


FILM_MAX_LAYERS = 12
FILM_TABLE_FLOATS = 6656


class FilmNet(C.Structure):
    _fields_ = [("hidden", C.c_int32), ("n_map", C.c_int32), ("n_film", C.c_int32),
                ("cond_dim", C.c_int32), ("x_dim", C.c_int32), ("out_dim", C.c_int32),
                ("map_w", C.c_void_p * FILM_MAX_LAYERS), ("map_b", C.c_void_p * FILM_MAX_LAYERS), ("map_ld", C.c_int32 * FILM_MAX_LAYERS),
                ("mo_w", C.c_void_p), ("mo_b", C.c_void_p), ("mo_ld", C.c_int32),
                ("film_w", C.c_void_p * FILM_MAX_LAYERS), ("film_b", C.c_void_p * FILM_MAX_LAYERS), ("film_ld", C.c_int32 * FILM_MAX_LAYERS),
                ("out_w", C.c_void_p), ("out_b", C.c_void_p), ("out_ld", C.c_int32)]


_film_layout = _sig("nsky_film_stream_layout", C.POINTER(FilmNet), C.c_int32, C.POINTER(C.c_int64), C.POINTER(C.c_int32))
_film_pack = _sig("nsky_film_pack", C.POINTER(FilmNet), C.c_int32, C.c_void_p, C.c_void_p, C.c_void_p)
_film_fwd = _sig("nsky_film_chain_fwd", C.POINTER(FilmNet), C.c_void_p, C.c_void_p, C.c_void_p, C.c_int32, C.c_void_p, C.c_int32, C.c_int32,
                 C.c_void_p, C.c_void_p, C.c_void_p, C.c_void_p, C.c_int32, C.c_void_p)


_film_bwd_film = _sig("nsky_film_chain_bwd_film", C.POINTER(FilmNet), C.c_void_p, C.c_void_p, C.c_int32, C.c_void_p, C.c_int32, C.c_void_p,
                      C.c_void_p, C.c_void_p, C.c_void_p, C.c_void_p, C.c_void_p, C.c_void_p, C.c_int32, C.c_void_p)
_film_bwd_map = _sig("nsky_film_chain_bwd_map", C.POINTER(FilmNet), C.c_void_p, C.c_void_p, C.c_int32, C.c_void_p, C.c_void_p, C.c_void_p,
                     C.c_void_p, C.c_void_p, C.c_int32, C.c_void_p, C.c_void_p)


_wgrad_native = _sig("nsky_wgrad_native", C.c_void_p, C.c_int32, C.c_void_p, C.c_int32, C.c_int32, C.c_void_p, C.c_int32, C.c_void_p,
                     C.c_void_p, C.c_float, C.c_void_p)


class WgradProblem(C.Structure):
    _fields_ = [("dZ", C.c_void_p), ("nnt_a", C.c_int32), ("X", C.c_void_p), ("nnt_b", C.c_int32), ("dW", C.c_void_p), ("ldw", C.c_int32),
                ("db", C.c_void_p), ("a_scale_max", C.c_void_p), ("b_scale", C.c_float),
                ("lda", C.c_int32), ("ldb", C.c_int32), ("width_a", C.c_int32), ("width_b", C.c_int32), ("bias_rows", C.c_int32),
                ("bias_row_mod", C.c_int32), ("b_scale_max", C.c_void_p)]


WGRAD_MAX_PROBLEMS = 16
_wgrad_native_batch = _sig("nsky_wgrad_native_batch", C.POINTER(WgradProblem), C.c_int32, C.c_int32, C.c_void_p)


def wgrad_problem(dZ, nnt_a, X, nnt_b, rows, dW, db=None, a_scale_max=None, b_scale=64.0, width_a=0, width_b=0, bias_row_mod=0,
                  b_scale_max=None) -> WgradProblem:
    wa, wb = width_a or 32 * nnt_a, width_b or 32 * nnt_b
    assert dW.stride(1) == 1 and dW.shape[0] >= wa and dW.shape[1] >= wb
    assert dZ.numel() >= film_rows(rows) * 32 * nnt_a and X.numel() >= film_rows(rows) * 32 * nnt_b
    return WgradProblem(ptr(dZ), nnt_a, ptr(X), nnt_b, ptr(dW), ld(dW), ptr(db), ptr(a_scale_max), float(b_scale), 0, 0, int(width_a), int(width_b), 0,
                        int(bias_row_mod), ptr(b_scale_max))


def wgrad_problem_rowmajor(dZ, n_out, X, k_in, rows, dW, db=None, bias_rows=0) -> WgradProblem:
    assert dW.stride(1) == 1 and dW.shape[0] >= n_out and dW.shape[1] >= k_in and n_out % 4 == 0 and k_in % 4 == 0
    assert dZ.shape[0] >= rows and X.shape[0] >= rows and ld(dZ) >= n_out and ld(X) >= k_in
    return WgradProblem(ptr(dZ), 0, ptr(X), 0, ptr(dW), ld(dW), ptr(db), None, 1.0, ld(dZ), ld(X), n_out, k_in, int(bias_rows), 0, None)


def wgrad_native_batch(problems, rows):
    for i in range(0, len(problems), WGRAD_MAX_PROBLEMS):
        chunk = problems[i:i + WGRAD_MAX_PROBLEMS]
        arr = (WgradProblem * len(chunk))(*chunk)
        check(_wgrad_native_batch(arr, len(chunk), rows, stream_ptr()), "nsky_wgrad_native_batch")


def wgrad_native(dZ, nnt_a, X, nnt_b, rows, dW, db=None, a_scale_max=None, b_scale=64.0):
    wgrad_problem(dZ, nnt_a, X, nnt_b, rows, dW, db, a_scale_max, b_scale)
    check(_wgrad_native(ptr(dZ), nnt_a, ptr(X), nnt_b, rows, ptr(dW), ld(dW), ptr(db), ptr(a_scale_max), float(b_scale), stream_ptr()),
          "nsky_wgrad_native")
    return dW


def film_supported(hidden, map_hidden, n_map, n_film, cond_dim, x_dim, out_dim) -> bool:
    return (hidden in (128, 256) and map_hidden == hidden and 1 <= n_map <= FILM_MAX_LAYERS and 1 <= n_film <= FILM_MAX_LAYERS
            and 1 <= cond_dim <= 320 and 1 <= x_dim <= 16 and 1 <= out_dim <= 4
            and n_map * hidden + 3 * n_film * hidden + 32 <= 6144)


def film_net(cond_dim, x_dim, out_dim, map_w, map_b, mo_w, mo_b, film_w, film_b, out_w, out_b) -> FilmNet:
    n = FilmNet(hidden=film_w[0].shape[0], n_map=len(map_w), n_film=len(film_w), cond_dim=cond_dim, x_dim=x_dim, out_dim=out_dim)
    for i, (w, b) in enumerate(zip(map_w, map_b)):
        n.map_w[i], n.map_b[i], n.map_ld[i] = ptr(w), ptr(b), ld(w)
    for i, (w, b) in enumerate(zip(film_w, film_b)):
        n.film_w[i], n.film_b[i], n.film_ld[i] = ptr(w), ptr(b), ld(w)
    n.mo_w, n.mo_b, n.mo_ld = ptr(mo_w), ptr(mo_b), ld(mo_w)
    n.out_w, n.out_b, n.out_ld = ptr(out_w), ptr(out_b), ld(out_w)
    return n


def film_stream_layout(net: FilmNet, direction: int = 0):
    nbytes, ntiles = C.c_int64(0), C.c_int32(0)
    check(_film_layout(C.byref(net), direction, C.byref(nbytes), C.byref(ntiles)), "nsky_film_stream_layout")
    return nbytes.value, ntiles.value


def film_pack(net: FilmNet, stream_buf, scales, direction: int = 0):
    check(_film_pack(C.byref(net), direction, ptr(stream_buf), ptr(scales), stream_ptr()), "nsky_film_pack")


_ray_points_fwd = _sig("nsky_ray_points_fwd", C.c_void_p, C.c_void_p, C.c_int32, C.c_float, C.c_void_p, C.c_int64, C.c_void_p, C.c_void_p)
_ray_points_bwd = _sig("nsky_ray_points_bwd", C.c_void_p, C.c_int32, C.c_float, C.c_void_p, C.c_int64, C.c_void_p, C.c_void_p)


def ray_points_fwd(origins, dirs, sign, t, out):
    n = origins.shape[0]
    assert origins.is_contiguous() and dirs.is_contiguous() and t.is_contiguous() and out.is_contiguous() and out.shape == (n, 3) and t.numel() == n
    check(_ray_points_fwd(ptr(origins), ptr(dirs), dirs.shape[0], float(sign), ptr(t), n, ptr(out), stream_ptr()), "nsky_ray_points_fwd")


def ray_points_bwd(dirs, sign, d_out, d_t):
    n = d_out.shape[0]
    assert dirs.is_contiguous() and d_out.is_contiguous() and d_t.is_contiguous() and d_t.numel() == n
    check(_ray_points_bwd(ptr(dirs), dirs.shape[0], float(sign), ptr(d_out), n, ptr(d_t), stream_ptr()), "nsky_ray_points_bwd")


_train_metrics = _sig("nsky_train_metrics", C.c_void_p, C.c_void_p, C.c_void_p, C.c_int64, C.c_float, C.c_void_p, C.c_void_p, C.c_void_p)


def train_metrics(pred, gt, mask, peak_sq, variance=None):
    n = pred.numel()
    assert pred.is_contiguous() and gt.is_contiguous() and gt.numel() == n and (mask is None or (mask.is_contiguous() and mask.numel() == n))
    assert pred.dtype == gt.dtype == torch.float32 and (mask is None or mask.dtype == torch.float32)
    out = torch.empty(3, device=pred.device)
    check(_train_metrics(ptr(pred), ptr(gt), ptr(mask), n, float(peak_sq), ptr(variance), ptr(out), stream_ptr()), "nsky_train_metrics")
    return out


_point_alphas_fwd = _sig("nsky_point_alphas_fwd", C.c_void_p, C.c_void_p, C.c_void_p, C.POINTER(C.c_float), C.c_void_p, C.c_float, C.c_int32,
                         C.c_void_p, C.c_void_p)
_point_alphas_bwd = _sig("nsky_point_alphas_bwd", C.c_void_p, C.c_void_p, C.c_void_p, C.POINTER(C.c_float), C.c_void_p, C.c_float, C.c_int32,
                         C.c_void_p, C.c_void_p, C.c_void_p, C.c_void_p, C.c_void_p)


def point_alphas_fwd(sdf, grad, dirs, gaps, variance, anneal, alphas):
    P = sdf.numel()
    assert sdf.is_contiguous() and grad.is_contiguous() and dirs.is_contiguous() and alphas.is_contiguous() and alphas.shape == (P, 3)
    g3 = (C.c_float * 3)(*[float(v) for v in gaps])
    check(_point_alphas_fwd(ptr(sdf), ptr(grad), ptr(dirs), g3, ptr(variance), float(anneal), P, ptr(alphas), stream_ptr()), "nsky_point_alphas_fwd")


def point_alphas_bwd(sdf, grad, dirs, gaps, variance, anneal, d_alphas, d_sdf, d_grad, d_variance):
    P = sdf.numel()
    assert d_alphas.is_contiguous() and d_sdf.is_contiguous() and d_grad.is_contiguous()
    g3 = (C.c_float * 3)(*[float(v) for v in gaps])
    check(_point_alphas_bwd(ptr(sdf), ptr(grad), ptr(dirs), g3, ptr(variance), float(anneal), P, ptr(d_alphas), ptr(d_sdf), ptr(d_grad),
                            ptr(d_variance), stream_ptr()), "nsky_point_alphas_bwd")


_sig_col_fwd = _sig("nsky_sigmoid_column_fwd", C.c_void_p, C.c_int32, C.c_int64, C.c_float, C.c_void_p, C.c_void_p)
_sig_col_bwd = _sig("nsky_sigmoid_column_bwd", C.c_void_p, C.c_int32, C.c_int64, C.c_float, C.c_void_p, C.c_void_p, C.c_void_p)


def sigmoid_column_fwd(raw, scale, t):
    assert raw.dim() == 2 and raw.stride(1) == 1 and t.is_contiguous() and t.numel() == raw.shape[0]
    check(_sig_col_fwd(ptr(raw), ld(raw), raw.shape[0], float(scale), ptr(t), stream_ptr()), "nsky_sigmoid_column_fwd")


def sigmoid_column_bwd(raw, scale, d_t, d_raw):
    assert d_raw.shape == raw.shape and d_raw.is_contiguous() and raw.is_contiguous() and d_t.is_contiguous()
    check(_sig_col_bwd(ptr(raw), ld(raw), raw.shape[0], float(scale), ptr(d_t), ptr(d_raw), stream_ptr()), "nsky_sigmoid_column_bwd")


_prop_fwd = _sig("nsky_proposal_mlp_fwd", C.c_void_p, C.c_int32, C.c_int64, C.c_int32, C.c_int32, C.c_void_p, C.c_int32, C.c_void_p, C.c_void_p,
                 C.c_void_p, C.c_void_p, C.c_void_p)
_prop_bwd = _sig("nsky_proposal_mlp_bwd", C.c_void_p, C.c_int32, C.c_int64, C.c_int32, C.c_int32, C.c_void_p, C.c_int32, C.c_void_p, C.c_void_p,
                 C.c_void_p, C.c_void_p, C.c_void_p, C.c_void_p, C.c_void_p, C.c_void_p, C.c_void_p, C.c_void_p)


def proposal_mlp_supported(in_dim: int, hidden: int) -> bool:
    return hidden == 16 and 1 <= in_dim <= 12


def proposal_mlp_fwd(feat, w0, b0, w1, b1, raw):
    P, in_dim = feat.shape[0], w0.shape[1]
    assert feat.stride(1) == 1 and w0.is_contiguous() and w1.is_contiguous() and raw.is_contiguous() and raw.numel() == P
    check(_prop_fwd(ptr(feat), ld(feat), P, in_dim, w0.shape[0], ptr(w0), ld(w0), ptr(b0), ptr(w1), ptr(b1), ptr(raw), stream_ptr()),
          "nsky_proposal_mlp_fwd")
# ... 61 lines not shown
    return SdfNet(in_dim=W0.shape[1], hidden=W0.shape[0], w0=ptr(W0), ld0=ld(W0), b0=ptr(b0), w1=ptr(W1), ld1=ld(W1), b1=ptr(b1),
                  w2=ptr(w2_row), b2=ptr(b2_elem), beta=float(beta))


def sdf_stream_layout(net: SdfNet, direction: int = 0):
    nbytes, ntiles = C.c_int64(0), C.c_int32(0)
    check(_sdf_layout(C.byref(net), direction, C.byref(nbytes), C.byref(ntiles)), "nsky_sdf_stream_layout")
    return nbytes.value, ntiles.value


def sdf_pack(net: SdfNet, stream_buf, table, direction: int = 0):
    check(_sdf_pack(C.byref(net), direction, ptr(stream_buf), ptr(table), stream_ptr()), "nsky_sdf_pack")


def sdf_chain_fwd(net: SdfNet, stream_buf, table, E, M, a0_save, a1_save, sdf):
    check(_sdf_fwd(C.byref(net), ptr(stream_buf), ptr(table), ptr(E), ld(E), M, ptr(a0_save), ptr(a1_save), ptr(sdf), stream_ptr()),
          "nsky_sdf_chain_fwd")
    return sdf


def sdf_chain_bwd(net: SdfNet, stream_buf, table, M, g_sdf, a0_save, a1_save, dz1, dz0, dE, dw2, db2, gmax):
    check(_sdf_bwd(C.byref(net), ptr(stream_buf), ptr(table), M, ptr(g_sdf), ptr(a0_save), ptr(a1_save), ptr(dz1), ptr(dz0),
                   ptr(dE), 0 if dE is None else ld(dE), ptr(dw2), ptr(db2), ptr(gmax), stream_ptr()), "nsky_sdf_chain_bwd")


CHAIN_MAX_LAYERS = 8


class ChainLayer(C.Structure):
    _fields_ = [("W", C.c_void_p), ("ld", C.c_int32), ("rows", C.c_int32), ("K", C.c_int32), ("transposed", C.c_int32)]


class FieldNet(C.Structure):
    _fields_ = [("in_dim", C.c_int32), ("npe", C.c_int32), ("beta", C.c_float),
                ("b0", C.c_void_p), ("b1", C.c_void_p), ("w_sdf", C.c_void_p), ("b_sdf", C.c_void_p), ("b2f", C.c_void_p),
                ("bc0", C.c_void_p), ("bc1", C.c_void_p), ("wc2", C.c_void_p), ("ldc2", C.c_int32), ("bc2", C.c_void_p)]


_chain_layout = _sig("nsky_chain_stream_layout", C.POINTER(ChainLayer), C.c_int32, C.POINTER(C.c_int64), C.POINTER(C.c_int32), C.POINTER(C.c_int32))
_chain_pack = _sig("nsky_chain_pack", C.POINTER(ChainLayer), C.c_int32, C.c_void_p, C.c_void_p, C.c_void_p)
_field_geo_fwd = _sig("nsky_field_geo_fwd", C.POINTER(FieldNet), C.c_void_p, C.c_void_p, C.c_int32, C.c_void_p, C.c_int32, C.c_int32, C.c_void_p,
                      C.c_void_p, C.c_void_p, C.c_void_p, C.c_void_p, C.c_void_p, C.c_void_p, C.c_void_p)
_field_col_fwd = _sig("nsky_field_colour_fwd", C.POINTER(FieldNet), C.c_void_p, C.c_void_p, C.c_int32, C.c_void_p, C.c_int32, C.c_int32, C.c_void_p,
                      C.c_void_p, C.c_void_p, C.c_void_p, C.c_void_p, C.c_void_p, C.c_void_p, C.c_void_p, C.c_void_p)
_field_col_bwd = _sig("nsky_field_colour_bwd", C.POINTER(FieldNet), C.c_void_p, C.c_void_p, C.c_int32, C.c_int32, C.c_void_p, C.c_void_p, C.c_void_p,
                      C.c_void_p, C.c_void_p, C.c_void_p, C.c_void_p, C.c_void_p, C.c_void_p, C.c_void_p, C.c_void_p, C.c_void_p)
_field_geo_bwd = _sig("nsky_field_geo_bwd", C.POINTER(FieldNet), C.c_void_p, C.c_void_p, C.c_int32, C.c_int32, C.c_void_p, C.c_void_p, C.c_void_p,
                      C.c_void_p, C.c_void_p, C.c_void_p, C.c_void_p, C.c_void_p, C.c_void_p, C.c_int32, C.c_void_p, C.c_void_p)
_native_wcolsum = _sig("nsky_native_weighted_colsum", C.c_void_p, C.c_int32, C.c_int32, C.c_void_p, C.c_int32, C.c_void_p, C.c_void_p, C.c_void_p,
                       C.c_int32, C.c_void_p, C.c_void_p)
_field_geo_fwd_dir = _sig("nsky_field_geo_fwd_dir", C.POINTER(FieldNet), C.c_void_p, C.c_void_p, C.c_int32, C.c_void_p, C.c_int32, C.c_int32,
                          C.c_void_p, C.c_void_p, C.c_void_p, C.c_void_p, C.c_void_p, C.c_void_p, C.c_void_p)
_field_geo_bwd_dir = _sig("nsky_field_geo_bwd_dir", C.POINTER(FieldNet), C.c_void_p, C.c_void_p, C.c_int32, C.c_int32, C.c_void_p, C.c_void_p,
                          C.c_void_p, C.c_void_p, C.c_void_p, C.c_void_p, C.c_void_p, C.c_int32, C.c_void_p, C.c_void_p)
_native_wcolsum_pair = _sig("nsky_native_weighted_colsum_pair", C.c_void_p, C.c_int32, C.c_int32, C.c_void_p, C.c_void_p, C.c_void_p, C.c_int32,
                            C.c_void_p, C.c_void_p)


def chain_layer(W, rows, K, transposed=False) -> ChainLayer:
    return ChainLayer(ptr(W), ld(W), int(rows), int(K), int(bool(transposed)))


def chain_pack(layers, device, buffers=None):
    arr = (ChainLayer * len(layers))(*layers)
    nbytes, ntiles, ngroups = C.c_int64(0), C.c_int32(0), C.c_int32(0)
    check(_chain_layout(arr, len(layers), C.byref(nbytes), C.byref(ntiles), C.byref(ngroups)), "nsky_chain_stream_layout")
    if buffers is not None:
        stream, scales = buffers(nbytes.value, max(ntiles.value, 4))
    else:
        stream = torch.zeros(nbytes.value, dtype=torch.uint8, device=device)
        scales = torch.empty(max(ntiles.value, 4), device=device)
    check(_chain_pack(arr, len(layers), ptr(stream), ptr(scales), stream_ptr()), "nsky_chain_pack")
    return stream, scales, ngroups.value


def field_supported(in_dim: int, hidden: int, geo_feat: int, hidden_colour: int, colour_in: int) -> bool:
    return hidden == 256 and geo_feat == 256 and hidden_colour == 256 and 68 <= in_dim <= 80 and in_dim % 4 == 0 and colour_in == 300


def field_net(in_dim, npe, beta, b0, b1, w_sdf, b_sdf, b2f=None, bc0=None, bc1=None, wc2=None, bc2=None) -> FieldNet:
    return FieldNet(in_dim=in_dim, npe=npe, beta=float(beta), b0=ptr(b0), b1=ptr(b1), w_sdf=ptr(w_sdf), b_sdf=ptr(b_sdf), b2f=ptr(b2f),
                    bc0=ptr(bc0), bc1=ptr(bc1), wc2=ptr(wc2), ldc2=0 if wc2 is None else ld(wc2), bc2=ptr(bc2))


def field_geo_fwd(net: FieldNet, pack, ET, N, a0q, a1q, Eq, a1max, sdf, grad, qmax=None):
    stream, scales, groups = pack
    check(_field_geo_fwd(C.byref(net), ptr(stream), ptr(scales), groups, ptr(ET), ld(ET), N, ptr(a0q), ptr(a1q), ptr(Eq), ptr(a1max), ptr(sdf),
                         ptr(grad), ptr(qmax), stream_ptr()), "nsky_field_geo_fwd")


def field_colour_fwd(net: FieldNet, pack, ET, N, a1q, a1max, a1v, feat, xpe, c0, c1, alb):
    stream, scales, groups = pack
    check(_field_col_fwd(C.byref(net), ptr(stream), ptr(scales), groups, ptr(ET), ld(ET), N, ptr(a1q), ptr(a1max), ptr(a1v), ptr(feat), ptr(xpe),
                         ptr(c0), ptr(c1), ptr(alb), stream_ptr()), "nsky_field_colour_fwd")


def field_colour_bwd(net: FieldNet, pack, N, g_alb, alb, c0, c1, dpc2, dpc1, dpc0, dfeat, dxpe, da1v, gmax):
    stream, scales, groups = pack
    check(_field_col_bwd(C.byref(net), ptr(stream), ptr(scales), groups, N, ptr(g_alb), ptr(alb), ptr(c0), ptr(c1), ptr(dpc2), ptr(dpc1), ptr(dpc0),
                         ptr(dfeat), ptr(dxpe), ptr(da1v), ptr(gmax), stream_ptr()), "nsky_field_colour_bwd")


def field_geo_bwd(net: FieldNet, pack, N, g_sdf, g_grad, da1v, dxpe, a0q, a1q, d1q, d0q, dET, gmax):
    stream, scales, groups = pack
    check(_field_geo_bwd(C.byref(net), ptr(stream), ptr(scales), groups, N, ptr(g_sdf), ptr(g_grad), ptr(da1v), ptr(dxpe), ptr(a0q), ptr(a1q),
                         ptr(d1q), ptr(d0q), ptr(dET), 0 if dET is None else ld(dET), ptr(gmax), stream_ptr()), "nsky_field_geo_bwd")


def native_weighted_colsum(X, nt, rows, out, bias=None, w4=None, n_out=1, g_sdf=None, g_grad=None):
    check(_native_wcolsum(ptr(X), nt, rows, ptr(w4), n_out, ptr(g_sdf), ptr(g_grad), ptr(out), ld(out) if out.dim() == 2 else out.shape[0],
                          ptr(bias), stream_ptr()), "nsky_native_weighted_colsum")


def field_geo_fwd_dir(net: FieldNet, pack, ET, N, a0q, a1q, Eq, sdf, cosv, qmax=None):
    stream, scales, groups = pack
    assert ET.shape[0] == 2 * N and sdf.numel() == N and cosv.numel() == N and a0q.shape[0] >= film_rows(2 * N) and a1q.shape[0] >= film_rows(2 * N)
    assert Eq is None or Eq.shape[0] >= film_rows(2 * N)
    check(_field_geo_fwd_dir(C.byref(net), ptr(stream), ptr(scales), groups, ptr(ET), ld(ET), N, ptr(a0q), ptr(a1q), ptr(Eq), ptr(sdf), ptr(cosv),
                             ptr(qmax), stream_ptr()), "nsky_field_geo_fwd_dir")


def field_geo_bwd_dir(net: FieldNet, pack, N, g_sdf, g_cos, a0q, a1q, d1q, d0q, dET, gmax):
    stream, scales, groups = pack
    assert (g_sdf is None or g_sdf.numel() == N) and (g_cos is None or g_cos.numel() == N) and (dET is None or dET.shape[0] == 2 * N)
    assert min(a0q.shape[0], a1q.shape[0], d1q.shape[0], d0q.shape[0]) >= film_rows(2 * N)
    check(_field_geo_bwd_dir(C.byref(net), ptr(stream), ptr(scales), groups, N, ptr(g_sdf), ptr(g_cos), ptr(a0q), ptr(a1q), ptr(d1q), ptr(d0q),
                             ptr(dET), 0 if dET is None else ld(dET), ptr(gmax), stream_ptr()), "nsky_field_geo_bwd_dir")


def native_weighted_colsum_pair(X, nt, rows, out, bias=None, g_sdf=None, g_cos=None):
    check(_native_wcolsum_pair(ptr(X), nt, rows, ptr(g_sdf), ptr(g_cos), ptr(out), ld(out) if out.dim() == 2 else out.shape[0], ptr(bias),
                               stream_ptr()), "nsky_native_weighted_colsum_pair")


def pair_native_to_rows(buf, N: int, width: int):
    return film_native_to_rows(buf, 2 * N, width).reshape(N, 2, width).permute(1, 0, 2)


def quad_native_to_rows(buf, N: int, width: int):
    return film_native_to_rows(buf, 4 * N, width).reshape(N, 4, width).permute(1, 0, 2)


def _ptr_array(ts, n):
    arr = (C.c_void_p * FILM_MAX_LAYERS)()
    for i in range(n):
        arr[i] = None if ts is None or ts[i] is None else ts[i].data_ptr()
    return arr


def film_keepless(hidden: int) -> str:
    return "registers" if hidden == 128 else "buffers"


def film_chain_fwd(net: FilmNet, stream_buf, scales, cond, x, M, h_save, z_save, y_save, res):
    check(_film_fwd(C.byref(net), ptr(stream_buf), ptr(scales), ptr(cond), ld(cond), ptr(x), ld(x), M,
                    _ptr_array(h_save, net.n_map), _ptr_array(z_save, net.n_film), _ptr_array(y_save, net.n_film), ptr(res), ld(res),
                    stream_ptr()), "nsky_film_chain_fwd")
    return res


def film_rows(M: int) -> int:
    return (M + 31) // 32 * 32


def film_native_to_rows(buf, M: int, width: int):
    R = film_rows(M) // 32
    return buf.reshape(R, width // 32, 4, 2, 32, 4).permute(0, 4, 1, 2, 3, 5).reshape(R * 32, width)[:M]


def film_rows_to_native(x, width: int):
    M = x.shape[0]
    R = film_rows(M) // 32
    full = x.new_zeros(R * 32, width)
    full[:M] = x[:, :width]
    return full.reshape(R, 32, width // 32, 4, 2, 4).permute(0, 2, 3, 4, 1, 5).contiguous().reshape(R * 32, width)


def film_chain_bwd_film(net: FilmNet, stream_buf, table, M, d_res, h_last, z_save, dz_save, dfp, dfp_rowmax, gmax, d_x=None):
    check(_film_bwd_film(C.byref(net), ptr(stream_buf), ptr(table), M, ptr(d_res), ld(d_res), ptr(h_last), _ptr_array(z_save, net.n_film),
                         _ptr_array(dz_save, net.n_film), ptr(dfp), ptr(dfp_rowmax), ptr(gmax), ptr(d_x), ld(d_x) if d_x is not None else 0,
                         stream_ptr()), "nsky_film_chain_bwd_film")


def film_chain_bwd_map(net: FilmNet, stream_buf, table, M, dfp, dfp_rowmax, h_save, dpre_save, d_cond, gmax):
    check(_film_bwd_map(C.byref(net), ptr(stream_buf), ptr(table), M, ptr(dfp), ptr(dfp_rowmax), _ptr_array(h_save, net.n_map),
                        _ptr_array(dpre_save, net.n_map), ptr(d_cond), ld(d_cond) if d_cond is not None else 0, ptr(gmax), stream_ptr()),
          "nsky_film_chain_bwd_map")


MC_TILE = 256
_mc_count = _sig("nsky_mc_count", C.c_void_p, C.c_int64, C.c_int64, C.c_int64, C.c_float, C.c_void_p, C.c_void_p)
_mc_vertices = _sig("nsky_mc_vertices", C.c_void_p, C.c_int64, C.c_int64, C.c_int64, C.c_float, C.c_float, C.c_float, C.c_float,
                    C.c_float, C.c_float, C.c_float, C.c_void_p, C.c_void_p, C.c_void_p, C.c_void_p, C.c_void_p)
_mc_faces = _sig("nsky_mc_faces", C.c_void_p, C.c_int64, C.c_int64, C.c_int64, C.c_float, C.c_void_p, C.c_void_p, C.c_void_p,
                 C.c_void_p, C.c_void_p)


def mc_count(volume, level: float, tile_counts):
    nx, ny, nz = volume.shape
    check(_mc_count(ptr(volume), nx, ny, nz, level, ptr(tile_counts), stream_ptr()), "nsky_mc_count")


def mc_vertices(volume, level: float, box_min, box_max, tile_vertex_offsets, base, edge_mask, vertices):
    nx, ny, nz = volume.shape
    check(_mc_vertices(ptr(volume), nx, ny, nz, level, *[float(v) for v in box_min], *[float(v) for v in box_max], ptr(tile_vertex_offsets),
                       ptr(base), ptr(edge_mask), ptr(vertices), stream_ptr()), "nsky_mc_vertices")


def mc_faces(volume, level: float, tile_face_offsets, base, edge_mask, faces):
    nx, ny, nz = volume.shape
    check(_mc_faces(ptr(volume), nx, ny, nz, level, ptr(tile_face_offsets), ptr(base), ptr(edge_mask), ptr(faces), stream_ptr()),
          "nsky_mc_faces")


MESH_KEY_BITS = 21
MESH_CELL_SUMS = 20
_GRID = (C.c_double, C.c_double, C.c_double, C.c_double)
_mesh_cell_keys = _sig("nsky_mesh_cell_keys", C.c_void_p, C.c_int64, *_GRID, C.c_void_p, C.c_void_p)
_mesh_cluster_count = _sig("nsky_mesh_cluster_count", C.c_void_p, C.c_int64, C.c_void_p, C.c_int64, *_GRID, C.c_void_p, C.c_void_p)
_mesh_vertex_cells = _sig("nsky_mesh_vertex_cells", C.c_void_p, C.c_void_p, C.c_int64, C.c_void_p, C.c_void_p)
_mesh_remap_faces = _sig("nsky_mesh_remap_faces", C.c_void_p, C.c_int64, C.c_void_p, C.c_int64, C.c_void_p, C.c_void_p, C.c_void_p)
_mesh_cluster_reduce = _sig("nsky_mesh_cluster_reduce", C.c_void_p, C.c_int64, C.c_void_p, C.c_int64, C.c_void_p, C.c_void_p, *_GRID,
                            C.c_void_p, C.c_void_p, C.c_int64, C.c_void_p, C.c_void_p, C.c_int32, C.c_void_p, C.c_void_p)
_mesh_cluster_solve = _sig("nsky_mesh_cluster_solve", C.c_void_p, C.c_void_p, C.c_int64, *_GRID, C.c_void_p, C.c_void_p, C.c_void_p,
                           C.c_void_p)
_mesh_flag_duplicates = _sig("nsky_mesh_flag_duplicates", C.c_void_p, C.c_int64, C.c_void_p, C.c_void_p, C.c_void_p, C.c_void_p)
_mesh_compact_faces = _sig("nsky_mesh_compact_faces", C.c_void_p, C.c_int64, C.c_void_p, C.c_void_p, C.c_int64, C.c_void_p, C.c_void_p)


def _mesh_grid(lo, h):
    return [float(lo[0]), float(lo[1]), float(lo[2]), float(h)]


def _typed(t, dtype, *shape):
    if t is not None and (t.dtype != dtype or tuple(t.shape) != shape or not t.is_contiguous()):
        raise ValueError(f"expected a contiguous {dtype} tensor shaped {shape}, got {t.dtype} {tuple(t.shape)}")
    return t


def mesh_cell_keys(vertices, lo, h: float, keys):
    V = vertices.shape[0]
    check(_mesh_cell_keys(ptr(_typed(vertices, torch.float32, V, 3)), V, *_mesh_grid(lo, h), ptr(_typed(keys, torch.int64, V)), stream_ptr()),
          "nsky_mesh_cell_keys")


def mesh_cluster_count(vertices, faces, lo, h: float, count):
    V, F = vertices.shape[0], faces.shape[0]
    check(_mesh_cluster_count(ptr(_typed(vertices, torch.float32, V, 3)), V, ptr(_typed(faces, torch.int32, F, 3)), F, *_mesh_grid(lo, h),
                              ptr(_typed(count, torch.int64, 1)), stream_ptr()), "nsky_mesh_cluster_count")


def mesh_vertex_cells(vertex_order, rank_sorted, vertex_cell):
    V = vertex_order.shape[0]
    check(_mesh_vertex_cells(ptr(_typed(vertex_order, torch.int64, V)), ptr(_typed(rank_sorted, torch.int64, V)), V,
                             ptr(_typed(vertex_cell, torch.int32, V)), stream_ptr()), "nsky_mesh_vertex_cells")


def mesh_remap_faces(faces, vertex_cell, corner_cells, face_keys):
    F, V = faces.shape[0], vertex_cell.shape[0]
    check(_mesh_remap_faces(ptr(_typed(faces, torch.int32, F, 3)), F, ptr(_typed(vertex_cell, torch.int32, V)), V,
                            ptr(_typed(corner_cells, torch.int32, F, 3)), ptr(_typed(face_keys, torch.int64, F)), stream_ptr()),
          "nsky_mesh_remap_faces")


def mesh_cluster_reduce(vertices, faces, normals, colours, lo, h: float, vertex_order, cell_start, sorted_corner_cells, corner_order,
                        cell_sums, group: int = 0):
    V, F, Cn = vertices.shape[0], faces.shape[0], cell_sums.shape[0]
    check(_mesh_cluster_reduce(ptr(_typed(vertices, torch.float32, V, 3)), V, ptr(_typed(faces, torch.int32, F, 3)), F,
                               ptr(_typed(normals, torch.float32, V, 3)), ptr(_typed(colours, torch.uint8, V, 3)), *_mesh_grid(lo, h),
                               ptr(_typed(vertex_order, torch.int64, V)), ptr(_typed(cell_start, torch.int64, Cn + 1)), Cn,
                               ptr(_typed(sorted_corner_cells, torch.int32, 3 * F)), ptr(_typed(corner_order, torch.int64, 3 * F)), group,
                               ptr(_typed(cell_sums, torch.float64, Cn, MESH_CELL_SUMS)), stream_ptr()), "nsky_mesh_cluster_reduce")


def mesh_cluster_solve(cell_sums, cell_keys, lo, h: float, vertices_out, normals_out=None, colours_out=None):
    Cn = cell_sums.shape[0]
    check(_mesh_cluster_solve(ptr(_typed(cell_sums, torch.float64, Cn, MESH_CELL_SUMS)), ptr(_typed(cell_keys, torch.int64, Cn)), Cn,
                              *_mesh_grid(lo, h), ptr(_typed(vertices_out, torch.float32, Cn, 3)), ptr(_typed(normals_out, torch.float32, Cn, 3)),
                              ptr(_typed(colours_out, torch.uint8, Cn, 3)), stream_ptr()), "nsky_mesh_cluster_solve")


def mesh_flag_duplicates(corner_cells, sorted_keys, face_order, keep):
    F = corner_cells.shape[0]
    check(_mesh_flag_duplicates(ptr(_typed(corner_cells, torch.int32, F, 3)), F, ptr(_typed(sorted_keys, torch.int64, F)),
                                ptr(_typed(face_order, torch.int64, F)), ptr(_typed(keep, torch.int32, F)), stream_ptr()),
          "nsky_mesh_flag_duplicates")


def mesh_compact_faces(corner_cells, keep, ends, faces_out):
    F, Fo = corner_cells.shape[0], faces_out.shape[0]
    check(_mesh_compact_faces(ptr(_typed(corner_cells, torch.int32, F, 3)), F, ptr(_typed(keep, torch.int32, F)), ptr(_typed(ends, torch.int64, F)),
                              Fo, ptr(_typed(faces_out, torch.int32, Fo, 3)), stream_ptr()), "nsky_mesh_compact_faces")


CC_STATUS_INDEX, CC_STATUS_LINK, CC_STATUS_FLATTEN = 1, 2, 4
_cc_link = _sig("nsky_cc_link", C.c_void_p, C.c_int64, C.c_int64, C.c_void_p, C.c_void_p, C.c_void_p)
_cc_flatten = _sig("nsky_cc_flatten", C.c_void_p, C.c_int64, C.c_void_p, C.c_int64, C.c_void_p, C.c_void_p, C.c_void_p, C.c_void_p)
_cc_select = _sig("nsky_cc_select", C.c_void_p, C.c_int64, C.c_int64, C.c_void_p, C.c_void_p, C.c_int64, C.c_void_p, C.c_void_p, C.c_void_p)
_cc_compact = _sig("nsky_cc_compact", C.c_void_p, C.c_void_p, C.c_void_p, C.c_int64, C.c_void_p, C.c_int64, C.c_void_p, C.c_void_p, C.c_void_p,
                   C.c_void_p, C.c_int64, C.c_int64, C.c_void_p, C.c_void_p, C.c_void_p, C.c_void_p, C.c_void_p)


def cc_link(faces, parent, status):
    F, V = faces.shape[0], parent.shape[0]
    check(_cc_link(ptr(_typed(faces, torch.int32, F, 3)), F, V, ptr(_typed(parent, torch.int32, V)), ptr(_typed(status, torch.int32, 1)),
                   stream_ptr()), "nsky_cc_link")


def cc_flatten(parent, faces, vertex_root, face_root, status):
    F, V = faces.shape[0], parent.shape[0]
    check(_cc_flatten(ptr(_typed(parent, torch.int32, V)), V, ptr(_typed(faces, torch.int32, F, 3)), F, ptr(_typed(vertex_root, torch.int32, V)),
                      ptr(_typed(face_root, torch.int32, F)), ptr(_typed(status, torch.int32, 1)), stream_ptr()), "nsky_cc_flatten")


def cc_select(faces, face_labels, keep_component, keep, vertex_used):
    F, V, Cn = faces.shape[0], vertex_used.shape[0], keep_component.shape[0]
    check(_cc_select(ptr(_typed(faces, torch.int32, F, 3)), F, V, ptr(_typed(face_labels, torch.int32, F)),
                     ptr(_typed(keep_component, torch.uint8, Cn)), Cn, ptr(_typed(keep, torch.uint8, F)),
                     ptr(_typed(vertex_used, torch.uint8, V)), stream_ptr()), "nsky_cc_select")


def cc_compact(vertices, normals, colours, faces, keep, face_ends, vertex_used, vertex_ends, vertices_out, normals_out, colours_out, faces_out):
    V, F, Vo, Fo = vertices.shape[0], faces.shape[0], vertices_out.shape[0], faces_out.shape[0]
    check(_cc_compact(ptr(_typed(vertices, torch.float32, V, 3)), ptr(_typed(normals, torch.float32, V, 3)), ptr(_typed(colours, torch.uint8, V, 3)),
                      V, ptr(_typed(faces, torch.int32, F, 3)), F, ptr(_typed(keep, torch.uint8, F)), ptr(_typed(face_ends, torch.int64, F)),
                      ptr(_typed(vertex_used, torch.uint8, V)), ptr(_typed(vertex_ends, torch.int64, V)), Vo, Fo,
                      ptr(_typed(vertices_out, torch.float32, Vo, 3)), ptr(_typed(normals_out, torch.float32, Vo, 3)),
                      ptr(_typed(colours_out, torch.uint8, Vo, 3)), ptr(_typed(faces_out, torch.int32, Fo, 3)), stream_ptr()), "nsky_cc_compact")


TEXTURE_MAX_SIZE = 16384
# ... 453 lines not shown
```

### neusky_amd/ops.py

```python
from __future__ import annotations

from typing import List, Optional, Sequence

import torch
import torch.nn.functional as F

from . import hip


_POLICIES = ("f32", "splith")
_FWD = {"splith": hip.PREC_F16X2}
_POLICY = "splith"
FWD_PRECISION = _FWD.get(_POLICY, hip.PREC_F32)
BWD_PRECISION = hip.PREC_F32


def set_precision_policy(policy: str) -> None:
    global FWD_PRECISION, _POLICY
    if policy not in _POLICIES:
        raise ValueError(policy)
    _POLICY = policy
    FWD_PRECISION = _FWD.get(policy, hip.PREC_F32)


# ... 493 lines not shown
        return out

    @staticmethod
    def backward(ctx, d_out):
        x, table = ctx.saved_tensors
        geom, mode, include_x, pe_freqs, pe_max_exp, tangents, need_dx, P, ldy = ctx.cfg
        if not ctx.needs_input_grad[1]:
            if not need_dx:
                return None, None, None, None, None, None, None, None, None, None
            dx = torch.empty(P, 3, device=x.device)
            hip.encode_bwd(geom, table, x, mode, include_x, pe_freqs, pe_max_exp, d_out.contiguous()[:P], None, None, dx)
            return dx, None, None, None, None, None, None, None, None, None
        d_out = d_out.contiguous()
        view = _sink_grad(ctx.sink, from_first_pass=True)
        accumulate = view is not None
        dtable = view.view_as(table) if accumulate else zeros_like(table)
        if ctx.dirs is not None:
            hip.encode_bwd_dir(geom, table, x, mode, include_x, pe_freqs, pe_max_exp, ctx.dirs, d_out[:P], d_out[P:], dtable)
            return None, (None if accumulate else dtable), None, None, None, None, None, None, None, None
        dx = torch.empty(P, 3, device=x.device) if need_dx else None
        dT = d_out[P:].view(3, P, ldy) if tangents else None
        hip.encode_bwd(geom, table, x, mode, include_x, pe_freqs, pe_max_exp, d_out[:P], dT, dtable, dx)
        return dx, (None if accumulate else dtable), None, None, None, None, None, None, None, None


_ACT = {"none": hip.EPI_NONE, "relu": hip.EPI_RELU}


class DenseFn(torch.autograd.Function):

    @staticmethod
    def forward(ctx, X, Wp, bp, n_out, act, need_dx):
        M, K = X.shape[0], Wp.shape[1]
        Y = torch.empty(M, n_out, device=X.device) if n_out == Wp.shape[0] else zeros(M, Wp.shape[0], device=X.device)
        fgemm(X, Wp, Y, M, n_out, K, bias=bp, epi=_ACT[act])
        ctx.save_for_backward(X, Wp, bp, Y)
        ctx.cfg = (n_out, act, need_dx)
        return Y

    @staticmethod
    def backward(ctx, dY):
        X, Wp, bp, Y = ctx.saved_tensors
        n_out, act, need_dx = ctx.cfg
        M, K = X.shape[0], Wp.shape[1]
        dZ = dY.contiguous()
        if act == "relu":
            dZ = torch.ops.aten.threshold_backward(dZ, Y, 0.0)
        dW = db = None
        if ctx.needs_input_grad[1] or ctx.needs_input_grad[2]:
            dW, db = grad_weight(dZ, X, M, n_out, K, Wp, bp)
        dX = None
        if need_dx:
            dX = torch.empty(M, K, device=X.device)
            frozen = not (ctx.needs_input_grad[1] or ctx.needs_input_grad[2])
            split_ok = frozen and _POLICY != "f32" and Wp.shape[0] % 32 == 0 and K > 64
            grad_input(dZ, Wp, M, K, Wp.shape[0], dX, precision=FROZEN_DX_PRECISION if split_ok else None)
        return dX, dW, db, None, None, None


def _film_fused_ok(x, cond, n_map, n_film, wb) -> bool:
    mw, _, _, _, fw, _, ow, _, _ = _film_unpack(wb, n_map, n_film)
    return (FWD_PRECISION == hip.PREC_F16X2 and ld(x) <= 16
            and hip.film_supported(fw[0].shape[0], mw[0].shape[0], n_map, n_film, mw[0].shape[1], fw[0].shape[1], ow.shape[0])
            and ld(x) >= fw[0].shape[1] and ld(cond) >= mw[0].shape[1])


def field_fused_ok(ET, W0, W1, W2, Wc0, Wc1) -> bool:
    return ET.shape[0] >= 4 and field_directional_ok(ld(ET), W0, W1, W2, Wc0, Wc1)


def field_directional_ok(ldE, W0, W1, W2, Wc0, Wc1) -> bool:
    return (FWD_PRECISION == hip.PREC_F16X2 and ldE == W0.shape[1]
            and hip.field_supported(W0.shape[1], W0.shape[0], W2.shape[0] - 4, Wc1.shape[0], Wc0.shape[1]))


def sdf_fused_ok(E, W0) -> bool:
    Hd, Kin = W0.shape
    return FWD_PRECISION == hip.PREC_F16X2 and hip.sdf_supported(Kin, Hd) and ld(E) >= Kin and ld(E) % 4 == 0


def film_apply(x, cond, n_map, n_film, train_weights, need_dcond, *wb):
    node = FilmChainFn if _film_fused_ok(x, cond, n_map, n_film, wb) else FilmLayersFn
    return node.apply(x, cond, n_map, n_film, train_weights, need_dcond, *wb)


def field_apply(ET, *args, directional=False):
    W0, _, W1, _, W2, _, Wc0, _, Wc1 = args[:9]
    if directional:
        if not field_directional_ok(ld(ET), W0, W1, W2, Wc0, Wc1):
            raise RuntimeError("field_apply: the directional mode exists on the fused field kernels only (see field_directional_ok)")
        beta = args[12]
        return FieldChainFn.apply(ET, *args[:12], beta, False, True)
    return (FieldChainFn if field_fused_ok(ET, W0, W1, W2, Wc0, Wc1) else SDFAlbedoFn).apply(ET, *args)


def sdf_value_apply(E, W0, *args):
    return (SdfChainFn if sdf_fused_ok(E, W0) else SdfLayersFn).apply(E, W0, *args)


_FILM_STREAMS: dict = {}


def forget_film_streams(wb) -> None:
    for key in [k for k, hit in _FILM_STREAMS.items() if hit[0] and wb and hit[0][0] is wb[0]]:
        del _FILM_STREAMS[key]


def _film_unpack(wb, n_map, n_film):
    mw = [wb[2 * i] for i in range(n_map)]
    mb = [wb[2 * i + 1] for i in range(n_map)]
    mwo, mbo = wb[2 * n_map], wb[2 * n_map + 1]
    o = 2 * n_map + 2
    fw = [wb[o + 2 * i] for i in range(n_film)]
    fb = [wb[o + 2 * i + 1] for i in range(n_film)]
    return mw, mb, mwo, mbo, fw, fb, wb[o + 2 * n_film], wb[o + 2 * n_film + 1], o


def _film_stream(wb, n_map, n_film, direction=0):
    key = (wb[0].data_ptr(), wb[0]._version, wb[-2].data_ptr(), n_map, n_film, direction)

    def pack():
        mw, mb, mwo, mbo, fw, fb, ow, ob, _ = _film_unpack(wb, n_map, n_film)
        net = hip.film_net(mw[0].shape[1], fw[0].shape[1], ow.shape[0], mw, mb, mwo, mbo, fw, fb, ow, ob)
        nbytes, _ = hip.film_stream_layout(net, direction)
        stream, table = _stream_buffers(("film", stable_id(wb[0]), n_map, n_film, direction), nbytes, hip.FILM_TABLE_FLOATS, wb[0].device)
        hip.film_pack(net, stream, table, direction)
        return net, stream, table
    return _prepared(_FILM_STREAMS, key, list(wb), pack)


class FilmChainFn(torch.autograd.Function):

    @staticmethod
    def forward(ctx, x, cond, n_map, n_film, train_weights, need_dcond, *wb):
        M = x.shape[0]
        dev = x.device
        mw, _, _, _, fw, _, ow, _, _ = _film_unpack(wb, n_map, n_film)
        H, Hm, n_out_p = fw[0].shape[0], mw[0].shape[0], ow.shape[0]
        save = any(ctx.needs_input_grad)
        train_w = train_weights and any(ctx.needs_input_grad[6:])
        keep_y = save and train_w
        net, stream, scales = _film_stream(wb, n_map, n_film)
        Mp = hip.film_rows(M)
        if keep_y:
            ys = [torch.empty(Mp, H, device=dev) for _ in range(n_film)]
        elif save and hip.film_keepless(H) == "registers":
            ys = None
        else:
            pp = [torch.empty(Mp, H, device=dev) for _ in range(min(2, n_film))]
            ys = [pp[i % len(pp)] for i in range(n_film)]
        hs = [torch.empty(Mp, Hm, device=dev) for _ in range(n_map)] if save else None
        zs = [torch.empty(Mp, H, device=dev) for _ in range(n_film)] if save else None
        res = torch.empty(M, n_out_p, device=dev)
        hip.film_chain_fwd(net, stream, scales, cond, x, M, hs, zs, ys, res)
        if not save:
            return res
        ctx.save_for_backward(x, cond, *hs, *(ys if keep_y else []), *zs, *wb)
        ctx.cfg = (n_map, n_film, train_w, need_dcond, M, H, Hm, x.requires_grad)
        ctx.sinks = [_sink_param(w) for w in wb]
        ctx.pad_sinks = [_sink_param(w, "pad") for w in wb]
        return res

    @staticmethod
    def backward(ctx, d_res):
        n_map, n_film, train_w, need_dcond, M, H, Hm, need_dx = ctx.cfg
        sv = ctx.saved_tensors
        x, cond = sv[0], sv[1]
        hs = list(sv[2:2 + n_map])
        n_ys = n_film if train_w else 0
        ys = list(sv[2 + n_map:2 + n_map + n_ys])
        zs = list(sv[2 + n_map + n_ys:2 + n_map + n_ys + n_film])
        wb = sv[2 + n_map + n_ys + n_film:]
        mw, mb, mwo, mbo, fw, fb, ow, ob, o = _film_unpack(wb, n_map, n_film)
        dev = x.device
        Mp = hip.film_rows(M)
        d_res = d_res.contiguous()
        net1, s1, t1 = _film_stream(wb, n_map, n_film, 1)
        net2, s2, t2 = _film_stream(wb, n_map, n_film, 2)
        dzs = [torch.empty(Mp, H, device=dev) for _ in range(n_film)] if train_w else None
        dfp = torch.empty(Mp, 2 * n_film * H, device=dev)
        rowmax = torch.empty(Mp, device=dev)
        gmax = zeros(n_film + 1 + n_map, device=dev)
        alloc = lambda t, w: (torch.empty if ld(t) == w else zeros)(M, ld(t), device=dev)
        d_x = alloc(x, fw[0].shape[1]) if need_dx else None
        hip.film_chain_bwd_film(net1, s1, t1, M, d_res, hs[-1], zs, dzs, dfp, rowmax, gmax[:n_film + 1], d_x)
        d_cond = alloc(cond, mw[0].shape[1]) if need_dcond else None
        want_map = need_dcond or train_w
        if train_w:
            dpres = [torch.empty(Mp, Hm, device=dev) for _ in range(n_map)]
        elif want_map and hip.film_keepless(Hm) == "buffers":
            dpres = [torch.empty(Mp, Hm, device=dev)] * n_map
        else:
            dpres = None
        if want_map:
            hip.film_chain_bwd_map(net2, s2, t2, M, dfp, rowmax, hs, dpres, d_cond, gmax[n_film + 1:])
        if not train_w:
            return (d_x, d_cond, None, None, None, None, *[None] * len(wb))
        grads, sunk = _carve_grads(wb, _sink_grads(ctx.sinks, from_first_pass=True))
        nt, ntm = H // 32, Hm // 32
        native = []

        def wgrad(dZ, X, n_out, k_in, like, bias_like, iw, a_nt, b_nt, smax, x_scale=64.0):
            if a_nt > 0 and b_nt > 0 and a_nt % 4 == 0 and b_nt % 4 == 0 and smax is not None:
                native.append(hip.wgrad_problem(dZ, a_nt, X, b_nt, M, grads[iw], grads[iw + 1], smax, x_scale))
            elif a_nt == 0 and b_nt > 0 and n_out <= 4 and dZ.dim() == 2 and dZ.shape[1] == 4 and dZ.is_contiguous():
                hip.native_weighted_colsum(X, b_nt, M, grads[iw], grads[iw + 1], w4=dZ, n_out=n_out)
            else:
                grad_weight(dZ, X, M, n_out, k_in, like, bias_like, acc=(grads[iw], grads[iw + 1]), a_native_nt=a_nt, b_native_nt=b_nt,
                            a_scale_max=smax)

        def launch():
            wgrad(d_res, ys[-1], ow.shape[0], H, ow, ob, o + 2 * n_film, 0, nt, None)
            for i in range(n_film - 1, 0, -1):
                wgrad(dzs[i], ys[i - 1], H, H, fw[i], fb[i], o + 2 * i, nt, nt, gmax[i:i + 1])
            wgrad(dzs[0], x, H, fw[0].shape[1], fw[0], fb[0], o, nt, 0, None)
            wgrad(dfp, hs[-1], 2 * n_film * H, Hm, mwo, mbo, 2 * n_map, 2 * n_film * nt, ntm, gmax[n_film:n_film + 1], 8.0)
            for l in range(n_map - 1, 0, -1):
                wgrad(dpres[l], hs[l - 1], Hm, Hm, mw[l], mb[l], 2 * l, ntm, ntm, gmax[n_film + 1 + l:n_film + 2 + l], 8.0)
            k0 = mw[0].shape[1]
            wgrad(dpres[0], cond, Hm, k0, mw[0], mb[0], 0, ntm, 0, gmax[n_film + 1:n_film + 2] if k0 > 64 else None)
            if native:
                hip.wgrad_native_batch(native, M)

        pads = _sink_grads(ctx.pad_sinks, from_first_pass=False, mark=False)
        if all(sunk[i] or pads[i] is not None for i in range(len(wb))):
            async_weight_gradients(launch, [d_res, x, cond, dfp, gmax, *ys, *hs, *dzs, *(dpres or [])])
            for i, view in enumerate(pads):
                if not sunk[i]:
                    shp = view.shape
                    _DEFERRED_PADS.append((grads[i][:shp[0], :shp[1]] if len(shp) == 2 else grads[i][:shp[0]], view))
                    sunk[i] = True
            _queue_end_of_pass()
        else:
            launch()
        return (d_x, d_cond, None, None, None, None, *[None if sunk[i] else g for i, g in enumerate(grads)])


class FilmLayersFn(torch.autograd.Function):

    @staticmethod
    def forward(ctx, x, cond, n_map, n_film, train_weights, need_dcond, *wb):
        M = x.shape[0]
        dev = x.device
        mw, mb, mwo, mbo, fw, fb, ow, ob, _ = _film_unpack(wb, n_map, n_film)
        H, Hm = fw[0].shape[0], mw[0].shape[0]
        n_out_p = ow.shape[0]
        save = any(ctx.needs_input_grad)
        if save:
            hs = [torch.empty(M, Hm, device=dev) for _ in range(n_map)]
            ys = [torch.empty(M, H, device=dev) for _ in range(n_film)]
            zs = [torch.empty(M, H, device=dev) for _ in range(n_film)]
        else:
            pp = [torch.empty(M, max(H, Hm), device=dev) for _ in range(2)]
            hs = [pp[i & 1][:, :Hm] for i in range(n_map)]
            ys = [pp[(n_map + i) & 1][:, :H] for i in range(n_film)]
            zs = [None] * n_film
        FP = torch.empty(M, 2 * n_film * H, device=dev)
        res = zeros(M, n_out_p, device=dev)
        h = cond
        for i in range(n_map):
            fgemm(h, mw[i], hs[i], M, Hm, mw[i].shape[1], bias=mb[i], epi=hip.EPI_LEAKY, p0=0.2)
            h = hs[i]
        fgemm(h, mwo, FP, M, 2 * n_film * H, Hm, bias=mbo)
        y = x
        for i in range(n_film):
            fgemm(y, fw[i], ys[i], M, H, fw[i].shape[1], bias=fb[i], epi=hip.EPI_FILM, p0=15.0, p1=30.0,
                  aux0=FP[:, i * H:(i + 1) * H], aux1=FP[:, (n_film + i) * H:(n_film + i + 1) * H], out1=zs[i])
            y = ys[i]
        fgemm(y, ow, res, M, n_out_p, H, bias=ob)
        if not save:
            return res
        ctx.save_for_backward(x, cond, FP, *hs, *ys, *zs, *wb)
        ctx.cfg = (n_map, n_film, train_weights, need_dcond, M, H, Hm, x.requires_grad)
        ctx.sinks = [_sink_param(w) for w in wb]
        return res

    @staticmethod
    def backward(ctx, d_res):
        n_map, n_film, train_w, need_dcond, M, H, Hm, need_dx = ctx.cfg
        train_w = train_w and any(ctx.needs_input_grad[6:])
        sv = ctx.saved_tensors
        x, cond, FP = sv[0], sv[1], sv[2]
        hs = list(sv[3:3 + n_map])
        ys = list(sv[3 + n_map:3 + n_map + n_film])
        zs = list(sv[3 + n_map + n_film:3 + n_map + 2 * n_film])
        wb = sv[3 + n_map + 2 * n_film:]
        mw, mb, mwo, mbo, fw, fb, ow, ob, o = _film_unpack(wb, n_map, n_film)
        dev = x.device
        d_res = d_res.contiguous()
        n_out_p = ow.shape[0]
        NF = 2 * n_film * H
        grads, sunk = [None] * len(wb), [False] * len(wb)
        if train_w:
            grads, sunk = _carve_grads(wb, _sink_grads(ctx.sinks, from_first_pass=True))
        acc = (lambda iw: (grads[iw], grads[iw + 1])) if train_w else (lambda iw: None)
        d_x = torch.empty(M, fw[0].shape[1], device=dev) if need_dx else None
        d_cond = torch.empty(M, mw[0].shape[1], device=dev) if need_dcond else None
        dFP = torch.empty(M, NF, device=dev)
        dZ, dZo = torch.empty(M, H, device=dev), torch.empty(M, H, device=dev)
        dpre, dpo = torch.empty(M, Hm, device=dev), torch.empty(M, Hm, device=dev)
        if train_w:
            grad_weight(d_res, ys[-1], M, n_out_p, H, ow, ob, acc=acc(o + 2 * n_film))
        i = n_film - 1
        grad_input(d_res, ow, M, H, n_out_p, dZ, epi=hip.EPI_BWD_FILM, p0=15.0, p1=30.0, aux0=zs[i],
                   aux1=FP[:, i * H:(i + 1) * H], aux2=FP[:, (n_film + i) * H:(n_film + i + 1) * H],
                   out1=dFP[:, i * H:(i + 1) * H], out2=dFP[:, (n_film + i) * H:(n_film + i + 1) * H])
        while True:
            y_in = ys[i - 1] if i > 0 else x
            k_in = fw[i].shape[1]
            if train_w:
                grad_weight(dZ, y_in, M, H, k_in, fw[i], fb[i], acc=acc(o + 2 * i))
            if i == 0:
                if d_x is not None:
                    grad_input(dZ, fw[0], M, k_in, H, d_x)
                break
            j = i - 1
            grad_input(dZ, fw[i], M, H, H, dZo, epi=hip.EPI_BWD_FILM, p0=15.0, p1=30.0, aux0=zs[j],
                       aux1=FP[:, j * H:(j + 1) * H], aux2=FP[:, (n_film + j) * H:(n_film + j + 1) * H],
                       out1=dFP[:, j * H:(j + 1) * H], out2=dFP[:, (n_film + j) * H:(n_film + j + 1) * H])
            dZ, dZo = dZo, dZ
            i = j
        if train_w:
            grad_weight(dFP, hs[-1], M, NF, Hm, mwo, mbo, acc=acc(2 * n_map))
        grad_input(dFP, mwo, M, Hm, NF, dpre, epi=hip.EPI_BWD_LEAKY, p0=0.2, aux0=hs[-1])
        for i in range(n_map - 1, -1, -1):
            h_in = hs[i - 1] if i > 0 else cond
            k_in = mw[i].shape[1]
            if train_w:
                grad_weight(dpre, h_in, M, Hm, k_in, mw[i], mb[i], acc=acc(2 * i))
            if i > 0:
                grad_input(dpre, mw[i], M, Hm, Hm, dpo, epi=hip.EPI_BWD_LEAKY, p0=0.2, aux0=hs[i - 1])
                dpre, dpo = dpo, dpre
            elif d_cond is not None:
                grad_input(dpre, mw[0], M, k_in, Hm, d_cond)
        return (d_x, d_cond, None, None, None, None, *[None if sunk[i] else g for i, g in enumerate(grads)])


class SDFAlbedoFn(torch.autograd.Function):
# ... 1011 lines not shown
```

Before: 54380 rays/s.

## Save FiLM frequency and sine argument in forward to skip backward recompute

The FiLM-SIREN forward kernel can now also store the per-layer frequency f and the sine argument for each element. A new backward kernel reads these saved values plus z instead of recomputing the FiLM and phase products. Its packed weight stream therefore holds only the transposed film weights, so the mapping-output tiles are no longer replayed with MFMA in backward. The saved path is on by default for hidden width 256 only (env-overridable). It adds two extra Mp×H fp32 buffers per FiLM layer, so forward writes and backward reads grow in exchange for fewer backward matrix products.

```diff
diff --git a/include/neusky_hip.h b/include/neusky_hip.h
--- a/include/neusky_hip.h
+++ b/include/neusky_hip.h
@@ -82,6 +82,14 @@
 int nsky_film_chain_bwd_map(const nsky_film_net* net, const void* stream_buf, const float* table, int32_t M, const float* dfp,
                             const float* dfp_rowmax, const float* const* h_save, float* const* dpre_save, float* d_cond,
                             int32_t ldcond, float* gmax, nsky_stream_t stream);
+int nsky_film_chain_fwd_saved(const nsky_film_net* net, const void* stream_buf, const float* table, const float* cond,
+                              int32_t ldcond, const float* x, int32_t ldx, int32_t M, float* const* h_save, float* const* z_save,
+                              float* const* y_save, float* const* f_save, float* const* arg_save, float* res, int32_t ldres,
+                              nsky_stream_t stream);
+int nsky_film_chain_bwd_film_saved(const nsky_film_net* net, const void* stream_buf, const float* table, int32_t M, const float* d_res,
+                                   int32_t ldres, const float* const* z_save, const float* const* f_save, const float* const* arg_save,
+                                   float* const* dz_save, float* dfp, float* dfp_rowmax, float* gmax, float* d_x, int32_t ldx,
+                                   nsky_stream_t stream);
 typedef struct {
   int32_t in_dim, hidden;
   const float* w0; int32_t ld0; const float* b0;
diff --git a/neusky_amd/csrc/film_chain.hip b/neusky_amd/csrc/film_chain.hip
--- a/neusky_amd/csrc/film_chain.hip
+++ b/neusky_amd/csrc/film_chain.hip
@@ -63,6 +63,11 @@
   n_tiles = n.n_film * NT * 2 + (n.n_film - 1) * NT + 1;
   total_groups = (long)n_tiles * Gh;
 }
+__host__ __device__ inline void bwd_film_saved_layout(const nsky_film_net& n, long& total_groups, int& n_tiles) {
+  const int NT = n.hidden / 32, Gh = groups_of(n.hidden);
+  n_tiles = (n.n_film - 1) * NT + 1;
+  total_groups = (long)n_tiles * Gh;
+}
 __host__ __device__ inline void bwd_map_layout(const nsky_film_net& n, long& total_groups, int& n_tiles) {
   const int NT = n.hidden / 32, Gh = groups_of(n.hidden);
   const int nkb = 2 * n.n_film * n.hidden / 64, ct = (n.cond_dim + 31) / 32;
@@ -88,6 +93,20 @@
     const int u = rem - 2 * NT;
     d.W = n.film_w[i]; d.ld = n.film_ld[i]; d.row0 = 32 * u; d.transposed = 1;
   }
+  return d;
+}
+
+__device__ inline TileDesc bwd_film_saved_tile(const nsky_film_net& n, int idx) {
+  TileDesc d;
+  const int NT = n.hidden / 32, H = n.hidden, Gh = groups_of(H);
+  d.group = (long)idx * Gh;
+  d.nrows = 32; d.K = H; d.k0 = 0; d.transposed = 1;
+  if (idx == (n.n_film - 1) * NT) {
+    d.W = n.film_w[0]; d.ld = n.film_ld[0]; d.row0 = 0; d.nrows = n.x_dim;
+    return d;
+  }
+  const int i = n.n_film - 1 - idx / NT, u = idx % NT;
+  d.W = n.film_w[i]; d.ld = n.film_ld[i]; d.row0 = 32 * u;
   return d;
 }
 
@@ -117,7 +136,8 @@
 __host__ __device__ inline void dir_layout(const nsky_film_net& n, int direction, long& total_groups, int& n_tiles) {
   if (direction == 0) { const Layout L = fwd_layout(n); total_groups = L.total_groups; n_tiles = L.n_tiles; }
   else if (direction == 1) bwd_film_layout(n, total_groups, n_tiles);
-  else bwd_map_layout(n, total_groups, n_tiles);
+  else if (direction == 2) bwd_map_layout(n, total_groups, n_tiles);
+  else bwd_film_saved_layout(n, total_groups, n_tiles);
 }
 
 __device__ inline void write_bias_table(const nsky_film_net& n, float* bl, int tid) {
@@ -146,7 +166,8 @@
     return;
   }
   const TileDesc d = direction == 0 ? fwd_tile(net, fwd_layout(net), blockIdx.x)
-                                    : (direction == 1 ? bwd_film_tile(net, blockIdx.x) : bwd_map_tile(net, blockIdx.x));
+                                    : (direction == 1 ? bwd_film_tile(net, blockIdx.x)
+                                                      : (direction == 2 ? bwd_map_tile(net, blockIdx.x) : bwd_film_saved_tile(net, blockIdx.x)));
   pack_tile(d, stream, table + BIAS_FLOATS, w, red);
 }
 
@@ -162,11 +183,13 @@
   float* h_save[MAXL];
   float* z_save[MAXL];
   float* y_save[MAXL];
+  float* f_save[MAXL];
+  float* arg_save[MAXL];
   float* res; int ldres;
 };
 
 
-template <int H, int KSC, bool KEEP_Y = true>
+template <int H, int KSC, bool KEEP_Y = true, bool SAVE_FA = false>
 __global__ __launch_bounds__(256, 1) void film_fwd_kernel(const FwdArgs a) {
   constexpr int NT = H / 32, KS = H / 16;
   __shared__ __attribute__((aligned(16))) unsigned char smem[RING_BYTES + (BIAS_FLOATS + SCALE_FLOATS) * 4];
@@ -280,6 +303,8 @@
     const float* bZ = bias_film + i * H;
     float* zblk = a.z_save[i] ? a.z_save[i] + (wave_live ? rt : 0) * NT * 1024 : nullptr;
     float* yblk = KEEP_Y ? a.y_save[i] + (wave_live ? rt : 0) * NT * 1024 : nullptr;
+    float* fblk = SAVE_FA ? a.f_save[i] + (wave_live ? rt : 0) * NT * 1024 : nullptr;
+    float* ablk = SAVE_FA ? a.arg_save[i] + (wave_live ? rt : 0) * NT * 1024 : nullptr;
     f16x8 nh[KEEP_Y ? 1 : KS], nl[KEEP_Y ? 1 : KS];
     for (int t = 0; t < NT; ++t) {
       f32x16 aF, aP, aZ;
@@ -297,7 +322,7 @@
       }
       const float iF = h_inv * sl[tile], iP = h_inv * sl[tile + 1], iZ = z_unscale * sl[tile + 2];
       tile += 3;
-      float zz[16], yy[16];
+      float zz[16], yy[16], ff[SAVE_FA ? 16 : 1], aa[SAVE_FA ? 16 : 1];
 #pragma unroll
       for (int g = 0; g < 4; ++g) {
         const int fo = 32 * t + 8 * g + 4 * h;
@@ -310,11 +335,17 @@
           const int r = 4 * g + q;
           const float F = fmaf(aF[r], iF, bf[q]), P = fmaf(aP[r], iP, bp[q]), z = fmaf(aZ[r], iZ, bz[q]);
           zz[r] = z;
-          yy[r] = sin_cw(fmaf(fmaf(15.0f, F, 30.0f), z, P));
+          const float f = fmaf(15.0f, F, 30.0f), arg = fmaf(f, z, P);
+          yy[r] = sin_cw(arg);
+          if constexpr (SAVE_FA) { ff[r] = f; aa[r] = arg; }
         }
       }
       if (wave_live) {
         if (zblk) store_tile_nt(zblk + t * 1024, lane, zz);
+        if constexpr (SAVE_FA) {
+          store_tile_nt(fblk + t * 1024, lane, ff);
+          store_tile_nt(ablk + t * 1024, lane, aa);
+        }
         if constexpr (KEEP_Y) store_tile(yblk + t * 1024, lane, yy);
       }
       if constexpr (!KEEP_Y) {
@@ -371,6 +402,8 @@
   const float* d_res; int ldres;
   const float* h_last;
   const float* z_save[MAXL];
+  const float* f_save[MAXL];
+  const float* arg_save[MAXL];
   float* dz_save[MAXL];
   float* dfp;
   float* dfp_rowmax;
@@ -577,6 +610,202 @@
   const long rt = (long)blockIdx.x * 4 + wave;
   if (rt < n_tiles) film_bwd4_tile<H, true, KEEP>(a, ws, bl, sl, wo, rt, lane);
   else film_bwd4_tile<H, false, KEEP>(a, ws, bl, sl, wo, 0, lane);
+  ws_close();
+}
+
+template <int N>
+__device__ __forceinline__ void hidden_wait12(f32x4 (&q)[12]) {
+  asm volatile("s_waitcnt vmcnt(%12)"
+               : "+v"(q[0]), "+v"(q[1]), "+v"(q[2]), "+v"(q[3]), "+v"(q[4]), "+v"(q[5]), "+v"(q[6]), "+v"(q[7]), "+v"(q[8]), "+v"(q[9]),
+                 "+v"(q[10]), "+v"(q[11])
+               : "n"(N) : "memory");
+}
+
+template <int H>
+__device__ __forceinline__ void film_bwd4s_request(const BwdFilmArgs& a, f32x4 (&q)[12], int i, int t, long rt, int lane) {
+  constexpr int NT = H / 32;
+  int toff = t * 1024;
+  asm volatile("" : "+s"(toff));
+  const float* zp = a.z_save[i] + rt * NT * 1024 + toff;
+  const float* fp = a.f_save[i] + rt * NT * 1024 + toff;
+  const float* ap = a.arg_save[i] + rt * NT * 1024 + toff;
+#pragma unroll
+  for (int k = 0; k < 12; ++k) q[k] = f32x4{0.f, 0.f, 0.f, 0.f};
+  hidden_load4_s<0>(q[0], zp, lane * 16);
+  hidden_load4_s<1024>(q[1], zp, lane * 16);
+  hidden_load4_s<2048>(q[2], zp, lane * 16);
+  hidden_load4_s<3072>(q[3], zp, lane * 16);
+  hidden_load4_s<0>(q[4], fp, lane * 16);
+  hidden_load4_s<1024>(q[5], fp, lane * 16);
+  hidden_load4_s<2048>(q[6], fp, lane * 16);
+  hidden_load4_s<3072>(q[7], fp, lane * 16);
+  hidden_load4_s<0>(q[8], ap, lane * 16);
+  hidden_load4_s<1024>(q[9], ap, lane * 16);
+  hidden_load4_s<2048>(q[10], ap, lane * 16);
+  hidden_load4_s<3072>(q[11], ap, lane * 16);
+}
+
+template <int H, bool KEEP, int N0>
+__device__ __forceinline__ void film_bwd4s_pass1(const BwdFilmArgs& a, f32x4 (&q)[2][12], f32x16 (&dY)[H / 32], int i, long rt, int lane,
+                                                 float& dz_max, float& fp_max) {
+  constexpr int NT = H / 32, NST = KEEP ? 12 : 8;
+  const int n_film = a.net.n_film;
+  float* dzp = KEEP ? a.dz_save[i] + rt * NT * 1024 : nullptr;
+  float* dFp = a.dfp + (rt * (2 * n_film * NT) + (long)i * NT) * 1024;
+  float* dPp = a.dfp + (rt * (2 * n_film * NT) + (long)(n_film + i) * NT) * 1024;
+  dz_max = 0.0f;
+#pragma unroll
+  for (int t = 0; t < NT; ++t) {
+    int toff = t * 1024;
+    asm volatile("" : "+s"(toff));
+    float *dzt = dzp + toff, *dFt = dFp + toff, *dPt = dPp + toff;
+    f32x4(&c)[12] = q[t & 1];
+    if (t + 1 < NT) film_bwd4s_request<H>(a, q[(t + 1) & 1], i, t + 1, rt, lane);
+    if (t == 0) hidden_wait12<N0>(c);
+    else if (t + 1 < NT) hidden_wait12<NST + 12>(c);
+    else hidden_wait12<NST>(c);
+#pragma unroll
+    for (int g = 0; g < 4; ++g) {
+      float dzv[4], dFv[4], dPv[4];
+#pragma unroll
+      for (int k = 0; k < 4; ++k) {
+        const int r = 4 * g + k;
+        const float z = c[g][k], f = c[4 + g][k];
+        const float gc = dY[t][r] * cos_cw(c[8 + g][k]);
+        dzv[k] = gc * f;
+        dFv[k] = 15.0f * gc * z;
+        dPv[k] = gc;
+        dY[t][r] = dzv[k];
+        dz_max = fmaxf(dz_max, fabsf(dzv[k]));
+        fp_max = fmaxf(fp_max, fmaxf(fabsf(dFv[k]), fabsf(gc)));
+      }
+      if constexpr (KEEP) {
+        stg4(dzt + (g * 256 + lane * 4), make_float4(dzv[0], dzv[1], dzv[2], dzv[3]));
+        stg4(dFt + (g * 256 + lane * 4), make_float4(dFv[0], dFv[1], dFv[2], dFv[3]));
+        stg4(dPt + (g * 256 + lane * 4), make_float4(dPv[0], dPv[1], dPv[2], dPv[3]));
+      } else {
+        *reinterpret_cast<f32x4*>(dFt + (g * 256 + lane * 4)) = f32x4{dFv[0], dFv[1], dFv[2], dFv[3]};
+        *reinterpret_cast<f32x4*>(dPt + (g * 256 + lane * 4)) = f32x4{dPv[0], dPv[1], dPv[2], dPv[3]};
+      }
+      asm volatile("" : "+v"(dz_max), "+v"(fp_max));
+    }
+  }
+}
+
+__device__ __forceinline__ float head_grad(const float4& dr, float w0, float w1, float w2, float w3) {
+  return fmaf(dr.w, w3, fmaf(dr.z, w2, fmaf(dr.x, w0, dr.y * w1)));
+}
+
+template <int H, bool ACTIVE, bool KEEP>
+__device__ __forceinline__ void film_bwd4s_tile(const BwdFilmArgs& a, WStream& ws, const float* sl, const float* wo, long rt, int lane) {
+  constexpr int NT = H / 32, KS = H / 16, GH = (KS + GSLABS - 1) / GSLABS, PW = 4;
+  static_assert(NT % 2 == 0, "tile 0 of every layer lands in buffer 0");
+  const nsky_film_net& net = a.net;
+  const int c = lane & 31, h = lane >> 5;
+  const long row = rt * 32 + c;
+  const bool live = ACTIVE && row < a.M;
+  const long rowc = row < a.M ? row : a.M - 1;
+  const int n_film = net.n_film;
+  f32x16 dY[NT];
+  f32x4 q[2][12];
+  if (ACTIVE) {
+    const float4 dr = ldg4(a.d_res + rowc * a.ldres);
+#pragma unroll
+    for (int t = 0; t < NT; ++t)
+#pragma unroll
+      for (int g = 0; g < 4; ++g) {
+        const int fo = 32 * t + 8 * g + 4 * h;
+        const float4 w0 = *reinterpret_cast<const float4*>(wo + fo), w1 = *reinterpret_cast<const float4*>(wo + H + fo);
+        const float4 w2 = *reinterpret_cast<const float4*>(wo + 2 * H + fo), w3 = *reinterpret_cast<const float4*>(wo + 3 * H + fo);
+        dY[t][4 * g] = head_grad(dr, w0.x, w1.x, w2.x, w3.x);
+        dY[t][4 * g + 1] = head_grad(dr, w0.y, w1.y, w2.y, w3.y);
+        dY[t][4 * g + 2] = head_grad(dr, w0.z, w1.z, w2.z, w3.z);
+        dY[t][4 * g + 3] = head_grad(dr, w0.w, w1.w, w2.w, w3.w);
+      }
+    asm volatile("s_waitcnt vmcnt(0)" ::: "memory");
+  } else {
+#pragma unroll
+    for (int t = 0; t < NT; ++t)
+#pragma unroll
+      for (int r = 0; r < 16; ++r) dY[t][r] = 0.0f;
+  }
+  float fp_max = 0.0f, dz_max = 0.0f;
+  int tile = 0;
+  auto split_dz = [&](int i, f16x8(&dh_)[KS], f16x8(&dl_)[KS]) __attribute__((always_inline)) {
+    float dz_inv = 1.0f;
+    if (ACTIVE) {
+      if constexpr (KEEP) publish_max(a.gmax + i, dz_max, live, true, lane);
+      const float s = row_scale(dz_max, dz_inv);
+#pragma unroll
+      for (int ks = 0; ks < KS; ++ks) {
+        float x8[8];
+#pragma unroll
+        for (int j = 0; j < 8; ++j) x8[j] = dY[ks >> 1][8 * (ks & 1) + j] * s;
+        split8(x8, dh_[ks], dl_[ks]);
+      }
+    }
+    return dz_inv;
+  };
+  if (ACTIVE) {
+    film_bwd4s_request<H>(a, q[0], n_film - 1, 0, rt, lane);
+    film_bwd4s_pass1<H, KEEP, 12>(a, q, dY, n_film - 1, rt, lane, dz_max, fp_max);
+  }
+  for (int i = n_film - 1; i > 0; --i) {
+    {
+      f16x8 dh_[KS], dl_[KS];
+      const float dz_inv = split_dz(i, dh_, dl_);
+#pragma unroll
+      for (int u = 0; u < NT; ++u) {
+        if (ACTIVE && u == NT - 1) film_bwd4s_request<H>(a, q[0], i - 1, 0, rt, lane);
+        f32x16 acc;
+        prod<KS, PW>(ws, ACTIVE, dh_, dl_, acc);
+        if (ACTIVE) {
+          const float inv = dz_inv * sl[tile];
+#pragma unroll
+          for (int r = 0; r < 16; ++r) dY[u][r] = acc[r] * inv;
+        }
+        ++tile;
+      }
+    }
+    if (ACTIVE) film_bwd4s_pass1<H, KEEP, GH * PW + 12>(a, q, dY, i - 1, rt, lane, dz_max, fp_max);
+  }
+  {
+    f16x8 dh_[KS], dl_[KS];
+    const float dz_inv = split_dz(0, dh_, dl_);
+    f32x16 acc;
+    prod<KS, PW>(ws, ACTIVE, dh_, dl_, acc);
+    if (ACTIVE && a.d_x && live) {
+      const float inv = dz_inv * sl[tile];
+#pragma unroll
+      for (int g = 0; g < 2; ++g)
+        if (8 * g + 4 * h < ((net.x_dim + 3) & ~3))
+          stg4(a.d_x + row * a.ldx + 8 * g + 4 * h, make_float4(acc[4 * g] * inv, acc[4 * g + 1] * inv, acc[4 * g + 2] * inv, acc[4 * g + 3] * inv));
+    }
+  }
+  if (ACTIVE) {
+    fp_max = fmaxf(fp_max, __shfl_xor(fp_max, 32, 64));
+    if (h == 0) a.dfp_rowmax[row] = fp_max;
+    publish_max(a.gmax + n_film, fp_max, live, true, lane);
+  }
+}
+
+template <int H, bool KEEP = true>
+__global__ __launch_bounds__(256, 1) void film_bwd4s_kernel(const BwdFilmArgs a) {
+  __shared__ __attribute__((aligned(16))) unsigned char smem[RING_BYTES + SCALE_FLOATS * 4 + 4 * H * 4];
+  float* sl = reinterpret_cast<float*>(smem + RING_BYTES);
+  float* wo = sl + SCALE_FLOATS;
+  const nsky_film_net& net = a.net;
+  const int tid = threadIdx.x, lane = tid & 63;
+  const int wave = __builtin_amdgcn_readfirstlane(tid >> 6);
+  for (int i = tid; i < SCALE_FLOATS; i += 256) sl[i] = a.table[BIAS_FLOATS + i];
+  for (int i = tid; i < 4 * H; i += 256) wo[i] = (i / H) < net.out_dim ? net.out_w[(long)(i / H) * net.out_ld + (i % H)] : 0.0f;
+  __syncthreads();
+  WStream ws;
+  ws_open(ws, a.stream, smem, wave, lane);
+  const long n_tiles = (a.M + 31) / 32;
+  const long rt = (long)blockIdx.x * 4 + wave;
+  if (rt < n_tiles) film_bwd4s_tile<H, true, KEEP>(a, ws, sl, wo, rt, lane);
+  else film_bwd4s_tile<H, false, KEEP>(a, ws, sl, wo, 0, lane);
   ws_close();
 }
 
@@ -799,7 +1028,7 @@
 
 extern "C" int nsky_film_stream_layout(const nsky_film_net* net, int32_t direction, int64_t* stream_bytes, int32_t* n_tiles) {
   if (int rc = check_net(net, "nsky_film_stream_layout")) return rc;
-  NSKY_CHECK_ARG(direction >= 0 && direction <= 2, "nsky_film_stream_layout: direction %d", direction);
+  NSKY_CHECK_ARG(direction >= 0 && direction <= 3, "nsky_film_stream_layout: direction %d", direction);
   long groups;
   int tiles;
   dir_layout(*net, direction, groups, tiles);
@@ -811,7 +1040,7 @@
 
 extern "C" int nsky_film_pack(const nsky_film_net* net, int32_t direction, void* stream_buf, float* table, nsky_stream_t stream) {
   if (int rc = check_net(net, "nsky_film_pack")) return rc;
-  NSKY_CHECK_ARG(direction >= 0 && direction <= 2 && stream_buf && table && ((uintptr_t)stream_buf % 16) == 0 && ((uintptr_t)table % 16) == 0, "nsky_film_pack: bad arguments");
+  NSKY_CHECK_ARG(direction >= 0 && direction <= 3 && stream_buf && table && ((uintptr_t)stream_buf % 16) == 0 && ((uintptr_t)table % 16) == 0, "nsky_film_pack: bad arguments");
   long groups;
   int tiles;
   dir_layout(*net, direction, groups, tiles);
@@ -822,9 +1051,10 @@
   return NSKY_OK;
 }
 
-extern "C" int nsky_film_chain_fwd(const nsky_film_net* net, const void* stream_buf, const float* table, const float* cond,
-                                   int32_t ldcond, const float* x, int32_t ldx, int32_t M, float* const* h_save, float* const* z_save,
-                                   float* const* y_save, float* res, int32_t ldres, nsky_stream_t stream) {
+namespace {
+int film_chain_fwd(const nsky_film_net* net, const void* stream_buf, const float* table, const float* cond, int32_t ldcond, const float* x,
+                   int32_t ldx, int32_t M, float* const* h_save, float* const* z_save, float* const* y_save, float* const* f_save,
+                   float* const* arg_save, float* res, int32_t ldres, nsky_stream_t stream) {
   if (int rc = check_net(net, "nsky_film_chain_fwd")) return rc;
   NSKY_CHECK_ARG(stream_buf && table && cond && x && res && M > 0, "nsky_film_chain_fwd: null operand / empty batch");
   NSKY_CHECK_ARG(ldcond % 4 == 0 && ldcond >= ((net->cond_dim + 3) & ~3) && ldx % 4 == 0 && ldx >= ((net->x_dim + 3) & ~3) && ldres >= 4 && ldres % 4 == 0,
@@ -839,28 +1069,55 @@
     a.h_save[l] = (h_save && l < net->n_map) ? h_save[l] : nullptr;
     a.z_save[l] = (z_save && l < net->n_film) ? z_save[l] : nullptr;
     a.y_save[l] = (y_save && l < net->n_film) ? y_save[l] : nullptr;
+    a.f_save[l] = (f_save && l < net->n_film) ? f_save[l] : nullptr;
+    a.arg_save[l] = (arg_save && l < net->n_film) ? arg_save[l] : nullptr;
   }
   const bool keep_y = a.y_save[0] != nullptr;
   NSKY_CHECK_ARG(keep_y || net->hidden == 128, "nsky_film_chain_fwd: NULL y_save needs hidden 128 (hidden %d: pass two ping-pong buffers)", net->hidden);
   for (int l = 0; l < net->n_film; ++l)
     NSKY_CHECK_ARG((a.y_save[l] != nullptr) == keep_y && ((uintptr_t)a.y_save[l] % 16) == 0, "nsky_film_chain_fwd: y_save[%d] missing / unaligned", l);
+  const bool save_fa = a.f_save[0] != nullptr;
+  for (int l = 0; l < net->n_film; ++l)
+    NSKY_CHECK_ARG((a.f_save[l] != nullptr) == save_fa && (a.arg_save[l] != nullptr) == save_fa && ((uintptr_t)a.f_save[l] % 16) == 0 &&
+                       ((uintptr_t)a.arg_save[l] % 16) == 0, "nsky_film_chain_fwd_saved: f_save / arg_save[%d] missing / unaligned", l);
   const dim3 grid(ceil_div(M, 128));
   const int ksc = ksteps_of(net->cond_dim);
-#define NSKY_FILM_FWD(HH, KK, KEEP) hipLaunchKernelGGL((film_fwd_kernel<HH, KK, KEEP>), grid, dim3(256), 0, (hipStream_t)stream, a)
-  if (net->hidden == 256) { if (ksc <= 4) NSKY_FILM_FWD(256, 4, true); else NSKY_FILM_FWD(256, 20, true); }
-  else if (keep_y) { if (ksc <= 4) NSKY_FILM_FWD(128, 4, true); else NSKY_FILM_FWD(128, 20, true); }
-  else { if (ksc <= 4) NSKY_FILM_FWD(128, 4, false); else NSKY_FILM_FWD(128, 20, false); }
+#define NSKY_FILM_FWD(HH, KK, KEEP)                                                                                              \
+  {                                                                                                                              \
+    if (save_fa) hipLaunchKernelGGL((film_fwd_kernel<HH, KK, KEEP, true>), grid, dim3(256), 0, (hipStream_t)stream, a);          \
+    else hipLaunchKernelGGL((film_fwd_kernel<HH, KK, KEEP, false>), grid, dim3(256), 0, (hipStream_t)stream, a);                 \
+  }
+  if (net->hidden == 256) { if (ksc <= 4) NSKY_FILM_FWD(256, 4, true) else NSKY_FILM_FWD(256, 20, true) }
+  else if (keep_y) { if (ksc <= 4) NSKY_FILM_FWD(128, 4, true) else NSKY_FILM_FWD(128, 20, true) }
+  else { if (ksc <= 4) NSKY_FILM_FWD(128, 4, false) else NSKY_FILM_FWD(128, 20, false) }
 #undef NSKY_FILM_FWD
   NSKY_CHECK_LAUNCH("nsky_film_chain_fwd");
   return NSKY_OK;
 }
-
-
-extern "C" int nsky_film_chain_bwd_film(const nsky_film_net* net, const void* stream_buf, const float* table, int32_t M, const float* d_res,
-                                        int32_t ldres, const float* h_last, const float* const* z_save, float* const* dz_save, float* dfp,
-                                        float* dfp_rowmax, float* gmax, float* d_x, int32_t ldx, nsky_stream_t stream) {
+}
+
+extern "C" int nsky_film_chain_fwd(const nsky_film_net* net, const void* stream_buf, const float* table, const float* cond,
+                                   int32_t ldcond, const float* x, int32_t ldx, int32_t M, float* const* h_save, float* const* z_save,
+                                   float* const* y_save, float* res, int32_t ldres, nsky_stream_t stream) {
+  return film_chain_fwd(net, stream_buf, table, cond, ldcond, x, ldx, M, h_save, z_save, y_save, nullptr, nullptr, res, ldres, stream);
+}
+
+extern "C" int nsky_film_chain_fwd_saved(const nsky_film_net* net, const void* stream_buf, const float* table, const float* cond,
+                                         int32_t ldcond, const float* x, int32_t ldx, int32_t M, float* const* h_save, float* const* z_save,
+                                         float* const* y_save, float* const* f_save, float* const* arg_save, float* res, int32_t ldres,
+                                         nsky_stream_t stream) {
+  NSKY_CHECK_ARG(f_save && arg_save, "nsky_film_chain_fwd_saved: null f_save / arg_save");
+  return film_chain_fwd(net, stream_buf, table, cond, ldcond, x, ldx, M, h_save, z_save, y_save, f_save, arg_save, res, ldres, stream);
+}
+
+
+namespace {
+int film_chain_bwd_film(const nsky_film_net* net, const void* stream_buf, const float* table, int32_t M, const float* d_res, int32_t ldres,
+                        const float* h_last, const float* const* z_save, const float* const* f_save, const float* const* arg_save,
+                        float* const* dz_save, float* dfp, float* dfp_rowmax, float* gmax, float* d_x, int32_t ldx, nsky_stream_t stream) {
   if (int rc = check_net(net, "nsky_film_chain_bwd_film")) return rc;
-  NSKY_CHECK_ARG(stream_buf && table && d_res && h_last && z_save && dfp && dfp_rowmax && gmax && M > 0, "nsky_film_chain_bwd_film: null operand / empty batch");
+  const bool saved = f_save != nullptr;
+  NSKY_CHECK_ARG(stream_buf && table && d_res && (h_last || saved) && z_save && dfp && dfp_rowmax && gmax && M > 0, "nsky_film_chain_bwd_film: null operand / empty batch");
   NSKY_CHECK_ARG(ldres >= 4 && ldres % 4 == 0 && ((uintptr_t)d_res % 16) == 0 && ((uintptr_t)h_last % 16) == 0 && ((uintptr_t)dfp % 16) == 0 &&
                      ((uintptr_t)stream_buf % 16) == 0 && ((uintptr_t)table % 16) == 0, "nsky_film_chain_bwd_film: alignment / ldres");
   NSKY_CHECK_ARG(net->hidden % 128 == 0, "nsky_film_chain_bwd_film: hidden %% 128");
@@ -870,19 +1127,44 @@
   if (d_x) NSKY_CHECK_ARG(ldx % 4 == 0 && ldx >= ((net->x_dim + 3) & ~3) && ldx <= 16 && ((uintptr_t)d_x % 16) == 0, "nsky_film_chain_bwd_film: d_x layout (ldx %d)", ldx);
   for (int l = 0; l < MAXL; ++l) {
     a.z_save[l] = l < net->n_film ? z_save[l] : nullptr;
+    a.f_save[l] = (saved && l < net->n_film) ? f_save[l] : nullptr;
+    a.arg_save[l] = (saved && l < net->n_film) ? arg_save[l] : nullptr;
     a.dz_save[l] = (dz_save && l < net->n_film) ? dz_save[l] : nullptr;
   }
+  for (int l = 0; saved && l < net->n_film; ++l)
+    NSKY_CHECK_ARG(a.f_save[l] && a.arg_save[l] && ((uintptr_t)a.f_save[l] % 16) == 0 && ((uintptr_t)a.arg_save[l] % 16) == 0,
+                   "nsky_film_chain_bwd_film_saved: f_save / arg_save[%d]", l);
   const bool keep = a.dz_save[0] != nullptr;
   for (int l = 0; l < net->n_film; ++l)
     NSKY_CHECK_ARG(a.z_save[l] && (a.dz_save[l] != nullptr) == keep && ((uintptr_t)a.z_save[l] % 16) == 0 && ((uintptr_t)a.dz_save[l] % 16) == 0, "nsky_film_chain_bwd_film: z_save / dz_save[%d]", l);
   a.full_wgs = a.tail_wgs = a.tail_k = 0;
   const dim3 grid(ceil_div(ceil_div(M, 32), 4));
-#define NSKY_FILM_BWD4(HH, KEEP) hipLaunchKernelGGL((film_bwd4_kernel<HH, KEEP>), grid, dim3(256), 0, (hipStream_t)stream, a)
-  if (net->hidden == 256) { if (keep) NSKY_FILM_BWD4(256, true); else NSKY_FILM_BWD4(256, false); }
-  else { if (keep) NSKY_FILM_BWD4(128, true); else NSKY_FILM_BWD4(128, false); }
+#define NSKY_FILM_BWD4(HH, KEEP)                                                                                       \
+  {                                                                                                                    \
+    if (saved) hipLaunchKernelGGL((film_bwd4s_kernel<HH, KEEP>), grid, dim3(256), 0, (hipStream_t)stream, a);          \
+    else hipLaunchKernelGGL((film_bwd4_kernel<HH, KEEP>), grid, dim3(256), 0, (hipStream_t)stream, a);                 \
+  }
+  if (net->hidden == 256) { if (keep) NSKY_FILM_BWD4(256, true) else NSKY_FILM_BWD4(256, false) }
+  else { if (keep) NSKY_FILM_BWD4(128, true) else NSKY_FILM_BWD4(128, false) }
 #undef NSKY_FILM_BWD4
   NSKY_CHECK_LAUNCH("nsky_film_chain_bwd_film");
   return NSKY_OK;
+}
+}
+
+extern "C" int nsky_film_chain_bwd_film(const nsky_film_net* net, const void* stream_buf, const float* table, int32_t M, const float* d_res,
+                                        int32_t ldres, const float* h_last, const float* const* z_save, float* const* dz_save, float* dfp,
+                                        float* dfp_rowmax, float* gmax, float* d_x, int32_t ldx, nsky_stream_t stream) {
+  NSKY_CHECK_ARG(h_last, "nsky_film_chain_bwd_film: null h_last");
+  return film_chain_bwd_film(net, stream_buf, table, M, d_res, ldres, h_last, z_save, nullptr, nullptr, dz_save, dfp, dfp_rowmax, gmax, d_x, ldx, stream);
+}
+
+extern "C" int nsky_film_chain_bwd_film_saved(const nsky_film_net* net, const void* stream_buf, const float* table, int32_t M, const float* d_res,
+                                              int32_t ldres, const float* const* z_save, const float* const* f_save,
+                                              const float* const* arg_save, float* const* dz_save, float* dfp, float* dfp_rowmax, float* gmax,
+                                              float* d_x, int32_t ldx, nsky_stream_t stream) {
+  NSKY_CHECK_ARG(f_save && arg_save, "nsky_film_chain_bwd_film_saved: null f_save / arg_save");
+  return film_chain_bwd_film(net, stream_buf, table, M, d_res, ldres, nullptr, z_save, f_save, arg_save, dz_save, dfp, dfp_rowmax, gmax, d_x, ldx, stream);
 }
 
 extern "C" int nsky_film_chain_bwd_map(const nsky_film_net* net, const void* stream_buf, const float* table, int32_t M, const float* dfp,
diff --git a/neusky_amd/hip.py b/neusky_amd/hip.py
--- a/neusky_amd/hip.py
+++ b/neusky_amd/hip.py
@@ -682,6 +682,7 @@
 
 FILM_MAX_LAYERS = 12
 FILM_TABLE_FLOATS = 6656
+FILM_SAVED_WIDTHS = (256,)
 
 
 class FilmNet(C.Structure):
@@ -701,6 +702,11 @@
 
 _film_bwd_film = _sig("nsky_film_chain_bwd_film", C.POINTER(FilmNet), C.c_void_p, C.c_void_p, C.c_int32, C.c_void_p, C.c_int32, C.c_void_p,
                       C.c_void_p, C.c_void_p, C.c_void_p, C.c_void_p, C.c_void_p, C.c_void_p, C.c_int32, C.c_void_p)
+_film_fwd_saved = _sig("nsky_film_chain_fwd_saved", C.POINTER(FilmNet), C.c_void_p, C.c_void_p, C.c_void_p, C.c_int32, C.c_void_p, C.c_int32,
+                       C.c_int32, C.c_void_p, C.c_void_p, C.c_void_p, C.c_void_p, C.c_void_p, C.c_void_p, C.c_int32, C.c_void_p)
+_film_bwd_film_saved = _sig("nsky_film_chain_bwd_film_saved", C.POINTER(FilmNet), C.c_void_p, C.c_void_p, C.c_int32, C.c_void_p, C.c_int32,
+                            C.c_void_p, C.c_void_p, C.c_void_p, C.c_void_p, C.c_void_p, C.c_void_p, C.c_void_p, C.c_void_p, C.c_int32,
+                            C.c_void_p)
 _film_bwd_map = _sig("nsky_film_chain_bwd_map", C.POINTER(FilmNet), C.c_void_p, C.c_void_p, C.c_int32, C.c_void_p, C.c_void_p, C.c_void_p,
                      C.c_void_p, C.c_void_p, C.c_int32, C.c_void_p, C.c_void_p)
 
@@ -1068,7 +1074,22 @@
     return "registers" if hidden == 128 else "buffers"
 
 
-def film_chain_fwd(net: FilmNet, stream_buf, scales, cond, x, M, h_save, z_save, y_save, res):
+def film_saved_operands(hidden: int) -> bool:
+    env = os.environ.get("NSKY_FILM_SAVED", "")
+    if env in ("0", "1"):
+        return env == "1"
+    if env:
+        return str(hidden) in env.split(",")
+    return hidden in FILM_SAVED_WIDTHS
+
+
+def film_chain_fwd(net: FilmNet, stream_buf, scales, cond, x, M, h_save, z_save, y_save, res, f_save=None, arg_save=None):
+    if f_save is not None or arg_save is not None:
+        check(_film_fwd_saved(C.byref(net), ptr(stream_buf), ptr(scales), ptr(cond), ld(cond), ptr(x), ld(x), M,
+                              _ptr_array(h_save, net.n_map), _ptr_array(z_save, net.n_film), _ptr_array(y_save, net.n_film),
+                              _ptr_array(f_save, net.n_film), _ptr_array(arg_save, net.n_film), ptr(res), ld(res), stream_ptr()),
+              "nsky_film_chain_fwd_saved")
+        return res
     check(_film_fwd(C.byref(net), ptr(stream_buf), ptr(scales), ptr(cond), ld(cond), ptr(x), ld(x), M,
                     _ptr_array(h_save, net.n_map), _ptr_array(z_save, net.n_film), _ptr_array(y_save, net.n_film), ptr(res), ld(res),
                     stream_ptr()), "nsky_film_chain_fwd")
@@ -1092,7 +1113,14 @@
     return full.reshape(R, 32, width // 32, 4, 2, 4).permute(0, 2, 3, 4, 1, 5).contiguous().reshape(R * 32, width)
 
 
-def film_chain_bwd_film(net: FilmNet, stream_buf, table, M, d_res, h_last, z_save, dz_save, dfp, dfp_rowmax, gmax, d_x=None):
+def film_chain_bwd_film(net: FilmNet, stream_buf, table, M, d_res, h_last, z_save, dz_save, dfp, dfp_rowmax, gmax, d_x=None, f_save=None,
+                        arg_save=None):
+    if f_save is not None or arg_save is not None:
+        check(_film_bwd_film_saved(C.byref(net), ptr(stream_buf), ptr(table), M, ptr(d_res), ld(d_res), _ptr_array(z_save, net.n_film),
+                                   _ptr_array(f_save, net.n_film), _ptr_array(arg_save, net.n_film), _ptr_array(dz_save, net.n_film),
+                                   ptr(dfp), ptr(dfp_rowmax), ptr(gmax), ptr(d_x), ld(d_x) if d_x is not None else 0, stream_ptr()),
+              "nsky_film_chain_bwd_film_saved")
+        return
     check(_film_bwd_film(C.byref(net), ptr(stream_buf), ptr(table), M, ptr(d_res), ld(d_res), ptr(h_last), _ptr_array(z_save, net.n_film),
                          _ptr_array(dz_save, net.n_film), ptr(dfp), ptr(dfp_rowmax), ptr(gmax), ptr(d_x), ld(d_x) if d_x is not None else 0,
                          stream_ptr()), "nsky_film_chain_bwd_film")
diff --git a/neusky_amd/ops.py b/neusky_amd/ops.py
--- a/neusky_amd/ops.py
+++ b/neusky_amd/ops.py
@@ -669,10 +669,14 @@
         hs = [torch.empty(Mp, Hm, device=dev) for _ in range(n_map)] if save else None
         zs = [torch.empty(Mp, H, device=dev) for _ in range(n_film)] if save else None
         res = torch.empty(M, n_out_p, device=dev)
-        hip.film_chain_fwd(net, stream, scales, cond, x, M, hs, zs, ys, res)
+        saved = save and hip.film_saved_operands(H)
+        fs = [torch.empty(Mp, H, device=dev) for _ in range(n_film)] if saved else None
+        ags = [torch.empty(Mp, H, device=dev) for _ in range(n_film)] if saved else None
+        hip.film_chain_fwd(net, stream, scales, cond, x, M, hs, zs, ys, res, fs, ags)
         if not save:
             return res
         ctx.save_for_backward(x, cond, *hs, *(ys if keep_y else []), *zs, *wb)
+        ctx.film_fa = (fs, ags)
         ctx.cfg = (n_map, n_film, train_w, need_dcond, M, H, Hm, x.requires_grad)
         ctx.sinks = [_sink_param(w) for w in wb]
         ctx.pad_sinks = [_sink_param(w, "pad") for w in wb]
@@ -681,6 +685,7 @@
     @staticmethod
     def backward(ctx, d_res):
         n_map, n_film, train_w, need_dcond, M, H, Hm, need_dx = ctx.cfg
+        fs, ags = ctx.film_fa
         sv = ctx.saved_tensors
         x, cond = sv[0], sv[1]
         hs = list(sv[2:2 + n_map])
@@ -692,7 +697,7 @@
         dev = x.device
         Mp = hip.film_rows(M)
         d_res = d_res.contiguous()
-        net1, s1, t1 = _film_stream(wb, n_map, n_film, 1)
+        net1, s1, t1 = _film_stream(wb, n_map, n_film, 1 if fs is None else 3)
         net2, s2, t2 = _film_stream(wb, n_map, n_film, 2)
         dzs = [torch.empty(Mp, H, device=dev) for _ in range(n_film)] if train_w else None
         dfp = torch.empty(Mp, 2 * n_film * H, device=dev)
@@ -700,7 +705,7 @@
         gmax = zeros(n_film + 1 + n_map, device=dev)
         alloc = lambda t, w: (torch.empty if ld(t) == w else zeros)(M, ld(t), device=dev)
         d_x = alloc(x, fw[0].shape[1]) if need_dx else None
-        hip.film_chain_bwd_film(net1, s1, t1, M, d_res, hs[-1], zs, dzs, dfp, rowmax, gmax[:n_film + 1], d_x)
+        hip.film_chain_bwd_film(net1, s1, t1, M, d_res, hs[-1], zs, dzs, dfp, rowmax, gmax[:n_film + 1], d_x, fs, ags)
         d_cond = alloc(cond, mw[0].shape[1]) if need_dcond else None
         want_map = need_dcond or train_w
         if train_w:
```

Measured after the change: 56100 rays/s (median of 6 runs). 1.03x the previous value.
